# sandyresearch/chipmunk

Measured on AMD Instinct MI355X. Metric: DiT denoise steps/sec at fixed sparsity, higher is better.
Workload: dtype bf16

## Files before the change

chipmunk_amd/_native.py:

```python
from __future__ import annotations

import ctypes
import os

_HERE = os.path.dirname(os.path.abspath(__file__))
LIB_PATH = os.environ.get("CHIPMUNK_HIP_LIB") or os.path.join(_HERE, "lib", "libchipmunk_hip.so")

SYMBOLS = [
    "chipmunk_last_error", "chipmunk_abi_version", "chipmunk_set_option", "chipmunk_set_random_seed",
    "chipmunk_csp_attn", "chipmunk_csp_attn_out", "chipmunk_csp_128_attn", "chipmunk_dense_attn", "chipmunk_dense_colsum_attn",
    "chipmunk_csp_mlp_mm1", "chipmunk_csp_mlp_mm1_scatter", "chipmunk_csp_mlp_mm1_fp8", "chipmunk_csp_mlp_mm2_and_scatter_add", "chipmunk_csp_scatter_add", "chipmunk_csp_mlp_mm2",
    "chipmunk_csp_mlp_mm1_ragged", "chipmunk_csp_mlp_mm1_scatter_ragged", "chipmunk_csp_mlp_mm1_fp8_ragged", "chipmunk_csp_mlp_mm2_ragged",
    "chipmunk_csp_mlp_mm2_and_scatter_add_ragged", "chipmunk_csp_scatter_add_ragged", "chipmunk_block_mean_ragged", "chipmunk_transpose16_pitched",
    "chipmunk_csp_mlp_mm1_batched", "chipmunk_csp_mlp_mm1_scatter_batched", "chipmunk_csp_mlp_mm1_fp8_batched", "chipmunk_csp_mlp_mm2_batched",
    "chipmunk_csp_mlp_mm2_and_scatter_add_batched", "chipmunk_csp_scatter_add_batched",
    "chipmunk_csp_mlp_mm1_glu", "chipmunk_csp_mlp_mm1_glu_batched", "chipmunk_csp_mlp_mm1_glu_fp8", "chipmunk_csp_mlp_mm1_glu_fp8_batched",
    "chipmunk_csp_mlp_mm1_act", "chipmunk_csp_mlp_mm1_act_batched", "chipmunk_csp_mlp_mm1_fp8_act", "chipmunk_csp_mlp_mm1_fp8_act_batched",
    "chipmunk_csp_mlp_mm2_w8", "chipmunk_csp_mlp_mm2_w8_batched",
    "chipmunk_csp_mlp_mm1_w8", "chipmunk_csp_mlp_mm1_w8_batched", "chipmunk_csp_mlp_mm1_w8_gm", "chipmunk_w8_linear",
    "chipmunk_csp_mlp_mm1_fp8_act_rs", "chipmunk_csp_mlp_mm1_fp8_act_rs_batched", "chipmunk_quantize_fp8_rowwise",
    "chipmunk_csp_mlp_mm1_act_gm", "chipmunk_csp_mlp_mm1_fp8_act_gm", "chipmunk_csp_mlp_mm1_fp8_act_rs_gm", "chipmunk_csp_mlp_mm1_glu_gm",
    "chipmunk_csp_mlp_mm1_glu_fp8_gm", "chipmunk_csp_scatter_add_gm", "chipmunk_transpose16_groups",
    "chipmunk_topk_indices", "chipmunk_topk_delta_indices", "chipmunk_topk_indices_p", "chipmunk_topk_delta_indices_p", "chipmunk_topk_group_delta_indices", "chipmunk_topk_group_delta_indices_p", "chipmunk_topk_mask", "chipmunk_topk_mask_p", "chipmunk_dense_colsum_topk_mask_p_strided", "chipmunk_mask_to_indices", "chipmunk_mask_to_sorted_indices", "chipmunk_packed_mask_to_indices", "chipmunk_mask_row_counts", "chipmunk_mask_to_ragged_indices", "chipmunk_copy_indices",
    "chipmunk_bitpack", "chipmunk_bitunpack", "chipmunk_transpose16", "chipmunk_block_mean", "chipmunk_quantize_fp8", "chipmunk_gather_rows", "chipmunk_qkv_split_norm", "chipmunk_split_heads_rownorm", "chipmunk_dense_colsum_topk_mask", "chipmunk_dense_attn_strided", "chipmunk_csp_attn_out_ragged", "chipmunk_compact_indices", "chipmunk_residual_ln_modulate", "chipmunk_residual_ln_modulate_f32", "chipmunk_dense_colsum_attn_strided", "chipmunk_dense_colsum_topk_mask_strided", "chipmunk_release_scratch", "chipmunk_big_scratch_fallbacks",
    "chipmunk_dense_attn_varlen", "chipmunk_dense_colsum_attn_varlen", "chipmunk_dense_colsum_topk_mask_varlen",
    "chipmunk_dense_colsum_topk_mask_p_varlen", "chipmunk_topk_mask_varlen", "chipmunk_topk_mask_p_varlen",
    "chipmunk_host_alloc", "chipmunk_host_free", "chipmunk_copy_d2h_async", "chipmunk_copy_h2d_async", "chipmunk_host_bytes",
]

_lib = None


def lib() -> ctypes.CDLL:
    global _lib
    if _lib is None:
        if not os.path.exists(LIB_PATH):
            raise ImportError(
                f"{LIB_PATH} is missing: build it with `python -m chipmunk_amd.build` (hipcc --offload-arch=gfx950). "
                "chipmunk_amd has no CPU fallback.")
        _lib = ctypes.CDLL(LIB_PATH)
        _lib.chipmunk_last_error.restype = ctypes.c_char_p
        _lib.chipmunk_abi_version.restype = ctypes.c_int
        vp, i, d = ctypes.c_void_p, ctypes.c_int, ctypes.c_double
        if hasattr(_lib, "chipmunk_topk_group_delta_indices"):
            _lib.chipmunk_topk_group_delta_indices.argtypes = [vp, vp, i, vp, vp, i, i, i, i, d, i, d, vp]
            _lib.chipmunk_topk_group_delta_indices_p.argtypes = [vp, vp, i, vp, vp, i, i, i, i, d, d, d, i, d, vp]
        for item in filter(None, os.environ.get("CHIPMUNK_AMD_OPTIONS", "").split(",")):
            name, _, val = item.partition("=")
            if _lib.chipmunk_set_option(name.strip().encode(), int(val)) != 0:
                raise ValueError(f"CHIPMUNK_AMD_OPTIONS: {_lib.chipmunk_last_error().decode()}")
    return _lib


def last_error() -> str:
    return lib().chipmunk_last_error().decode()


def check(rc: int, what: str) -> None:
    if rc != 0:
# ... 59 lines not shown
```

chipmunk_amd/csrc/attn.hip:

```cpp
#include "common.h"
#include "attn_params.h"
#include <type_traits>

namespace {

constexpr int QG = 192;
constexpr int QW = 48;
constexpr int KVT = 32;
constexpr int NST = 4;
constexpr int KRING = 8;
constexpr int HD = 128;
constexpr int TILE_BYTES = KVT * HD * 2;
constexpr float SCALE_LOG2E = 0.08838834764f * 1.44269504089f;
constexpr int NSTV = NST + 1;
constexpr int KEY_RING_OFF = (NST + NSTV) * TILE_BYTES;
constexpr int CS_OFF = KEY_RING_OFF + KRING * 256;
constexpr int ATTN_LDS_BYTES = CS_OFF + 2 * 2 * 4 * KVT * 4;

__device__ __forceinline__ f32x4 mfma16(bf16x8 a, bf16x8 b, f32x4 c) {
    return __builtin_amdgcn_mfma_f32_16x16x32_bf16(a, b, c, 0, 0, 0);
}

#ifdef ATTN_PROF
__device__ unsigned long long g_attn_prof[8 * 8];
// ... 1217 lines not shown
    if (use_colsum64(B, H, Nq, Nk)) return chipmunk_colsum64_launch(p, st);
    return launch_attn<false, false, false, true>(p, st);
}

extern "C" int chipmunk_dense_colsum_attn_strided(const void *q, const void *k, const void *v, const int64_t q_strides[3],
                                                  const int64_t k_strides[3], const int64_t v_strides[3], const float *pin,
                                                  void *o, const int64_t *o_strides, void *cs, float *l, int B, int H, int Nq,
                                                  int Nk, int cs_stride, void *stream) {
    return dense_colsum_attn_impl(q, k, v, q_strides, k_strides, v_strides, pin, o, o_strides, cs, l, nullptr, B, H, Nq, Nk, cs_stride,
                                  stream);
}

extern "C" int chipmunk_dense_colsum_attn_varlen(const void *q, const void *k, const void *v, const int64_t q_strides[3],
                                                 const int64_t k_strides[3], const int64_t v_strides[3], const float *pin,
                                                 void *o, const int64_t *o_strides, void *cs, float *l, const int32_t *k_lens, int B,
                                                 int H, int Nq, int Nk, int cs_stride, void *stream) {
    return dense_colsum_attn_impl(q, k, v, q_strides, k_strides, v_strides, pin, o, o_strides, cs, l, k_lens, B, H, Nq, Nk, cs_stride,
                                  stream);
}

extern "C" int chipmunk_dense_colsum_attn(const void *q, const void *k, const void *v, const int64_t q_strides[3],
                                          const int64_t k_strides[3], const int64_t v_strides[3], const float *pin,
                                          void *o, void *cs, float *l, int B, int H, int Nq, int Nk, int cs_stride,
                                          void *stream) {
    return chipmunk_dense_colsum_attn_strided(q, k, v, q_strides, k_strides, v_strides, pin, o, nullptr, cs, l, B, H, Nq, Nk,
                                              cs_stride, stream);
}

static int dense_colsum_topk_mask_impl(const void *q, const void *k, const void *v, const int64_t q_strides[3],
                                       const int64_t k_strides[3], const int64_t v_strides[3], const float *pin, void *o,
                                       const int64_t *o_strides, float *l, int B, int H, int Nq, int Nk, const void *static_mask,
                                       int64_t static_stride, int static_rows, const void *group_flags, void *mask,
                                       int topk, double random_amount, bool mass, double top_p, int k_min, void *stream,
                                       const int32_t *klens = nullptr) {
    if (int e = check_common(q, k, v, o, B, H, Nq, Nk)) return e;
    CM_CHECK(l && pin && mask, "dense_colsum_topk_mask: p / l / mask missing");
    if (int e = check_strides(q_strides, "q")) return e;
    if (int e = check_strides(k_strides, "k")) return e;
    if (int e = check_strides(v_strides, "v")) return e;
    hipStream_t st = (hipStream_t)stream;
    if (!use_dense64(B, H, Nq, Nk) || chipmunk_get_option("attn_fused_colsum") == 2 || (Nk & 3) || Nk > CHIPMUNK_TOPK_MASK_MAX_N)
        return CHIPMUNK_ERR_UNSUPPORTED;
    AttnParams p = {};
    p.q = (const uint16_t *)q, p.k = (const uint16_t *)k, p.v = (const uint16_t *)v, p.o = (uint16_t *)o;
    for (int i = 0; i < 3; ++i) p.qs[i] = q_strides[i], p.ks[i] = k_strides[i], p.vs[i] = v_strides[i];
    CM_CHECK((int64_t)Nk * p.ks[2] * 2 < (1ll << 32) && (int64_t)Nk * p.vs[2] * 2 < (1ll << 32),
             "attention: one head's K or V spans more than 4 GiB (32-bit DMA offsets)");
    if (int e = output_strides(p.os, o_strides, H, Nq)) return e;
    p.l_out = l, p.p_in = pin, p.cs = nullptr, p.cs_stride = 0, p.klens = klens;
    p.B = B, p.H = H, p.Nq = Nq, p.Nk = Nk, p.G = (Nq + QG - 1) / QG;
    p.o_scale = 1.f;
    uint16_t *part = (uint16_t *)chipmunk_big_scratch(st, chipmunk_colsum_part_bytes(B, H, Nq, Nk));
    if (!part) return CHIPMUNK_ERR_UNSUPPORTED;
    if (int e = chipmunk_dense64_colsum_launch(p, part, st)) return e;
    const int nrb = ((Nq + 255) / 256) * 2;
    if (mass)
        return chipmunk_topk_mask_p_parts(part, chipmunk_colsum_part_stride(Nk), nrb, p.G, Nq, static_mask, static_stride, static_rows, group_flags, mask,
                                          B * H * p.G, Nk, topk, top_p, k_min, random_amount, st, klens, H * p.G);
    return chipmunk_topk_mask_parts(part, chipmunk_colsum_part_stride(Nk), nrb, p.G, Nq, static_mask, static_stride, static_rows, group_flags, mask, B * H * p.G, Nk,
                                    topk, random_amount, st, klens, H * p.G);
}

extern "C" int chipmunk_dense_colsum_topk_mask_strided(const void *q, const void *k, const void *v, const int64_t q_strides[3],
                                               const int64_t k_strides[3], const int64_t v_strides[3], const float *pin, void *o,
                                               const int64_t *o_strides, float *l, int B, int H, int Nq, int Nk, const void *static_mask,
                                               int64_t static_stride, int static_rows, const void *group_flags, void *mask,
                                               int topk, double random_amount, void *stream) {
    return dense_colsum_topk_mask_impl(q, k, v, q_strides, k_strides, v_strides, pin, o, o_strides, l, B, H, Nq, Nk, static_mask, static_stride,
                                       static_rows, group_flags, mask, topk, random_amount, false, 0.0, 0, stream);
}

extern "C" int chipmunk_dense_colsum_topk_mask_p_strided(const void *q, const void *k, const void *v, const int64_t q_strides[3],
                                                 const int64_t k_strides[3], const int64_t v_strides[3], const float *pin, void *o,
                                                 const int64_t *o_strides, float *l, int B, int H, int Nq, int Nk, const void *static_mask,
                                                 int64_t static_stride, int static_rows, const void *group_flags, void *mask,
                                                 int topk, double random_amount, double top_p, int k_min, void *stream) {
    CM_CHECK(top_p > 0.0 && top_p <= 1.0, "dense_colsum_topk_mask_p: top_p must be in (0, 1] (got %g)", top_p);
    CM_CHECK(k_min >= 0, "dense_colsum_topk_mask_p: k_min must be >= 0 (got %d)", k_min);
    return dense_colsum_topk_mask_impl(q, k, v, q_strides, k_strides, v_strides, pin, o, o_strides, l, B, H, Nq, Nk, static_mask, static_stride,
                                       static_rows, group_flags, mask, topk, random_amount, true, top_p, k_min, stream);
}

extern "C" int chipmunk_dense_colsum_topk_mask(const void *q, const void *k, const void *v, const int64_t q_strides[3],
                                               const int64_t k_strides[3], const int64_t v_strides[3], const float *pin, void *o,
                                               float *l, int B, int H, int Nq, int Nk, const void *static_mask,
                                               int64_t static_stride, int static_rows, const void *group_flags, void *mask,
                                               int topk, double random_amount, void *stream) {
    return chipmunk_dense_colsum_topk_mask_strided(q, k, v, q_strides, k_strides, v_strides, pin, o, nullptr, l, B, H, Nq, Nk,
                                                   static_mask, static_stride, static_rows, group_flags, mask, topk, random_amount,
                                                   stream);
}

extern "C" int chipmunk_dense_colsum_topk_mask_varlen(const void *q, const void *k, const void *v, const int64_t q_strides[3],
                                                      const int64_t k_strides[3], const int64_t v_strides[3], const float *pin, void *o,
                                                      const int64_t *o_strides, float *l, const int32_t *k_lens, int B, int H, int Nq,
                                                      int Nk, const void *static_mask, int64_t static_stride, int static_rows,
                                                      const void *group_flags, void *mask, int topk, double random_amount, void *stream) {
    return dense_colsum_topk_mask_impl(q, k, v, q_strides, k_strides, v_strides, pin, o, o_strides, l, B, H, Nq, Nk, static_mask, static_stride,
                                       static_rows, group_flags, mask, topk, random_amount, false, 0.0, 0, stream, k_lens);
}

extern "C" int chipmunk_dense_colsum_topk_mask_p_varlen(const void *q, const void *k, const void *v, const int64_t q_strides[3],
                                                        const int64_t k_strides[3], const int64_t v_strides[3], const float *pin, void *o,
                                                        const int64_t *o_strides, float *l, const int32_t *k_lens, int B, int H, int Nq,
                                                        int Nk, const void *static_mask, int64_t static_stride, int static_rows,
                                                        const void *group_flags, void *mask, int topk, double random_amount, double top_p,
                                                        int k_min, void *stream) {
    CM_CHECK(top_p > 0.0 && top_p <= 1.0, "dense_colsum_topk_mask_p: top_p must be in (0, 1] (got %g)", top_p);
    CM_CHECK(k_min >= 0, "dense_colsum_topk_mask_p: k_min must be >= 0 (got %d)", k_min);
    return dense_colsum_topk_mask_impl(q, k, v, q_strides, k_strides, v_strides, pin, o, o_strides, l, B, H, Nq, Nk, static_mask, static_stride,
                                       static_rows, group_flags, mask, topk, random_amount, true, top_p, k_min, stream, k_lens);
}
```

chipmunk_amd/csrc/attn_params.h:

```cpp
#pragma once
#include <stdint.h>
#include <hip/hip_runtime.h>

struct AttnParams {
    const uint16_t *q, *k, *v;
    uint16_t *o;
    const uint16_t *o_in;
    int64_t qs[3], ks[3], vs[3], os[3];
    const int32_t *indices, *counts;
    const int64_t *idx_off;
    float *l_out;
    const float *p_in;
    uint16_t *cs;
    int cs_stride;
    int B, H, Nq, Nk, G, idx_stride;
    float o_scale;
    int split_full, nsplit;
    float *ws;
    int32_t *tickets;
    const int32_t *plan;
    int xcd_chunks;
    const float *kmax;
    uint16_t *cs_part;
    int cs_pstride;
    int probe;
    const int32_t *klens;
};

__device__ __forceinline__ int item_nk(const int32_t *klens, int b, int Nk) {
    if (!klens) return Nk;
    const int n = klens[b];
    return n < 1 ? 1 : (n < Nk ? n : Nk);
}


int chipmunk_csp64_launch(const AttnParams &p, int inplace, int grid, hipStream_t stream);
int chipmunk_dense64_colsum_launch(const AttnParams &p, uint16_t *part, hipStream_t stream);
int chipmunk_topk_mask_parts(const uint16_t *part, int part_stride, int nrb, int groups_per_bh, int Nq, const void *static_mask, int64_t static_stride,
                             int static_rows, const void *group_flags, void *mask, int rows, int n, int k, double random_amount,
                             hipStream_t stream, const int32_t *klens = nullptr, int seq_rows = 0);
int chipmunk_topk_mask_p_parts(const uint16_t *part, int part_stride, int nrb, int groups_per_bh, int Nq, const void *static_mask, int64_t static_stride,
                               int static_rows, const void *group_flags, void *mask, int rows, int n, int k, double top_p, int k_min,
                               double random_amount, hipStream_t stream, const int32_t *klens = nullptr, int seq_rows = 0);
size_t chipmunk_colsum_part_bytes(int B, int H, int Nq, int Nk);
int chipmunk_colsum_part_stride(int Nk);
int chipmunk_colsum64_launch(const AttnParams &p, hipStream_t stream);
int chipmunk_csp96_launch(const AttnParams &p, int inplace, int grid, hipStream_t stream);
const float *chipmunk_knorm_max(const uint16_t *k, const int64_t ks[3], int B, int H, int Nk, hipStream_t stream, const int32_t *klens = nullptr);

__host__ __device__ inline int colsum_part_rows(int j, int nwg, int &r0, int &r1) {
    const int a = (3 * j) >> 2, w0 = 3 * j - 4 * a;
    r0 = 2 * a + (w0 ? 1 : 0);
    r1 = 2 * (a + 1);
    return (w0 >= 2 && a + 1 < nwg) ? 2 : 1;
}

struct IndexRow {
    const int32_t *ptr;
    int width;
};
__device__ __forceinline__ IndexRow index_row(const AttnParams &p, int64_t item) {
    if (p.idx_off) {
        const int64_t o = p.idx_off[item];
        return {p.indices + o, (int)(p.idx_off[item + 1] - o)};
    }
    return {p.indices + item * p.idx_stride, p.idx_stride};
}
```

chipmunk_amd/csrc/indexed_io.hip:

```cpp
#include "common.h"
#include "attn_params.h"

namespace {

__device__ __forceinline__ uint32_t wave_incl_scan(uint32_t x) {
    x += (uint32_t)__builtin_amdgcn_update_dpp(0, (int)x, 0x111, 0xf, 0xf, true);
    x += (uint32_t)__builtin_amdgcn_update_dpp(0, (int)x, 0x112, 0xf, 0xf, true);
    x += (uint32_t)__builtin_amdgcn_update_dpp(0, (int)x, 0x114, 0xf, 0xf, true);
    x += (uint32_t)__builtin_amdgcn_update_dpp(0, (int)x, 0x118, 0xf, 0xf, true);
    x += (uint32_t)__builtin_amdgcn_update_dpp(0, (int)x, 0x142, 0xa, 0xf, false);
    x += (uint32_t)__builtin_amdgcn_update_dpp(0, (int)x, 0x143, 0xc, 0xf, false);
    return x;
}
struct M2IParams {
    const uint8_t *mask;
    int32_t *indices;
    int32_t *counts;
    int n, pad_n, multiple_of;
    const int64_t *offsets;
};

template <bool PACKED, bool SORTED = false, bool RAGGED = false>
__global__ __launch_bounds__(256) void mask_to_indices_kernel(const M2IParams p) {
    extern __shared__ __attribute__((aligned(16))) unsigned char smem[];
// ... 190 lines not shown
};

template <bool PACKED>
__global__ __launch_bounds__(256) void mask_row_counts_kernel(const RowCountParams p) {
    const int lane = threadIdx.x & 63;
    const int64_t row = (int64_t)blockIdx.x * 4 + (threadIdx.x >> 6);
    if (row >= p.rows) return;
    const int nbytes = PACKED ? p.n >> 3 : p.n;
    const uint8_t *src = p.mask + (PACKED ? (row * p.n) >> 3 : row * p.n);
    auto set_in_byte = [](uint32_t b) { return PACKED ? (uint32_t)__popc(b) : (uint32_t)(b != 0); };
    auto set_in_word = [](uint32_t x) {
        if constexpr (!PACKED) x = (x | (x >> 1) | (x >> 2) | (x >> 3) | (x >> 4) | (x >> 5) | (x >> 6) | (x >> 7)) & 0x01010101u;
        return (uint32_t)__popc(x);
    };
    const int head = min(nbytes, (int)((16 - ((uintptr_t)src & 15)) & 15));
    uint32_t cnt = lane < head ? set_in_byte(src[lane]) : 0u;
    const int nvec = (nbytes - head) >> 4;
    const u32x4 *vec = (const u32x4 *)(src + head);
#pragma unroll 4
    for (int i = lane; i < nvec; i += 64) {
        const u32x4 x = vec[i];
        cnt += set_in_word(x[0]) + set_in_word(x[1]) + set_in_word(x[2]) + set_in_word(x[3]);
    }
    const int tail = head + (nvec << 4) + lane;
    if (tail < nbytes) cnt += set_in_byte(src[tail]);
    const int64_t kept = (uint32_t)__builtin_amdgcn_readlane((int)wave_incl_scan(cnt), 63);
    if (lane == 0) {
        const int64_t padded = ((kept + p.multiple_of - 1) / p.multiple_of) * p.multiple_of;
        p.counts[row] = (int32_t)padded;
        p.lengths[row] = (min(padded, (int64_t)p.pad_n) + 31) / 32 * 32;
    }
}

struct TopkParams {
    const void *act;
    void *cache;
    int32_t *indices;
    int32_t *counts;
    int rows, cols, multiple_of;
    float quantile, random_amount;
    uint32_t salt;
    int group_rows, src_rows, groups;
};

template <typename T>
__device__ __forceinline__ float load_as_float(const T *p, int i);
template <>
__device__ __forceinline__ float load_as_float<uint16_t>(const uint16_t *p, int i) { return bf16_bits_to_f32(p[i]); }
template <>
__device__ __forceinline__ float load_as_float<_Float16>(const _Float16 *p, int i) { return (float)p[i]; }
template <>
__device__ __forceinline__ float load_as_float<float>(const float *p, int i) { return p[i]; }

template <typename T>
__device__ __forceinline__ float round_to(float x);
template <>
__device__ __forceinline__ float round_to<uint16_t>(float x) { return round_bf16(x); }
template <>
__device__ __forceinline__ float round_to<_Float16>(float x) { return (float)(_Float16)x; }
template <>
__device__ __forceinline__ float round_to<float>(float x) { return x; }

__device__ __forceinline__ float hash_uniform(uint32_t row, uint32_t col, uint32_t salt) {
    uint32_t x = (row * 0x9E3779B9u ^ (col + 0x7F4A7C15u) * 0x85EBCA6Bu) + salt * 0xC2B2AE35u;
    x ^= x >> 16, x *= 0x7feb352du, x ^= x >> 15, x *= 0x846ca68bu, x ^= x >> 16;
    return (float)(x >> 8) * (1.0f / 16777216.0f);
// ... 359 lines not shown
    CM_CHECK(mask && indices && (RAGGED ? (const void *)offsets : (const void *)counts), "mask_to_indices: null pointer");
    CM_CHECK(rows >= 0 && n > 0 && pad_n >= n && multiple_of > 0, "mask_to_indices: bad sizes rows=%lld n=%d pad_n=%d multiple_of=%d",
             (long long)rows, n, pad_n, multiple_of);
    CM_CHECK(rows < (1ll << 31), "mask_to_indices: too many rows");
    if (PACKED) CM_CHECK(n % 8 == 0, "packed_mask_to_indices: n must be a multiple of 8 (got %d)", n);
    const size_t lds = m2i_lds_bytes(n, SORTED);
    CM_CHECK(lds <= 160 * 1024, "mask_to_indices: row length %d needs %zu B of LDS (> 160 KiB)", n, lds);
    if (rows == 0) return CHIPMUNK_OK;
    auto kern = mask_to_indices_kernel<PACKED, SORTED, RAGGED>;
    if (lds > 64 * 1024) (void)hipFuncSetAttribute((const void *)kern, hipFuncAttributeMaxDynamicSharedMemorySize, (int)lds);
    M2IParams p = {(const uint8_t *)mask, indices, counts, n, pad_n, multiple_of, offsets};
    hipLaunchKernelGGL(kern, dim3((unsigned)rows), dim3(256), lds, (hipStream_t)stream, p);
    CM_LAUNCH_CHECK();
    return CHIPMUNK_OK;
}


struct TopkMaskParams {
    const uint16_t *cs;
    const uint8_t *stat;
    const uint8_t *groups;
    uint8_t *mask;
    int64_t cs_stride, stat_stride;
    int rows, n, k, stat_rows;
    float random_amount;
    uint32_t salt;
    const uint16_t *parts;
    int64_t pstride;
    int nrb, ngroups, nq;
    float top_p;
    int k_min;
    const int32_t *klens;
    int seq_rows;
};

__device__ __forceinline__ int topk_mask_row_len(const TopkMaskParams &p, int row) {
    if (!p.klens) return p.n;
    const int v = p.klens[row / p.seq_rows];
    return v < 1 ? 1 : (v < p.n ? v : p.n);
}
struct RowCut {
    int tid, step;
    uint32_t keep0, keep1;
};
__device__ __forceinline__ RowCut row_cut(int nv) {
    const int rem = nv & 3;
    RowCut c;
    c.tid = rem ? ((nv - 1) >> 2) & 1023 : -1;
    c.step = (nv - 1) >> 12;
    c.keep0 = rem == 1 ? 0xffffu : 0xffffffffu;
    c.keep1 = rem == 3 ? 0xffffu : (rem ? 0u : 0xffffffffu);
    return c;
}

__device__ __forceinline__ float key_value(uint32_t key) { return __uint_as_float((key ^ 0x8000u) << 16); }
__device__ __forceinline__ void add_mass2(float &m, uint32_t kw, float flo) {
    const uint32_t kx = kw ^ 0x80008000u;
    const float a = __uint_as_float(kx << 16), b = __uint_as_float(kx & 0xffff0000u);
    m += a >= flo ? a : 0.f;
    m += b >= flo ? b : 0.f;
}

__device__ __forceinline__ int topp_count(float total, float target, float above, int gt, int eq, uint32_t thr, int k, int k_min) {
    int kp = 0;
    if (total > 0.f && target > 0.f) {
        const float v = key_value(thr);
        float t = __builtin_ceilf((target - above) / v);
        t = t >= 1.f ? t : 1.f;
        kp = gt + (t < (float)eq ? (int)t : eq);
    }
    const int s = kp > k_min ? kp : k_min;
    return s < k ? s : k;
}

__device__ __forceinline__ uint32_t bf16_key(uint32_t u) {
    return (u & 0x8000u) ? (~u & 0xffffu) : (u | 0x8000u);
}

template <int KPT, bool ALIGNED, bool PARTS = false, bool MASS = false>
__global__ __launch_bounds__(1024) void topk_mask_kernel(const TopkMaskParams p) {
    constexpr int NV = KPT / 4;
    __shared__ int wave_cnt[16];
    const int tid = threadIdx.x, lane = tid & 63, w = tid >> 6;
    const int row = blockIdx.x;
    const int n = p.n;
    const int nv = topk_mask_row_len(p, row);
    const uint16_t *x = nullptr;
    int prow = 1;
    int64_t row1 = 0;
    if constexpr (PARTS) {
        const int bh = row / p.ngroups, g = row - bh * p.ngroups;
        int r0, r1;
        prow = colsum_part_rows(g, p.nrb / 2, r0, r1);
        x = p.parts + ((int64_t)bh * p.nrb + r0) * p.pstride;
        row1 = (int64_t)(r1 - r0) * p.pstride;
    } else {
        x = p.cs + (int64_t)row * p.cs_stride;
    }
    const uint32_t lane_off8 = 8u * (uint32_t)tid;
    const uint32_t lane_off4 = 4u * (uint32_t)tid;
    uint32_t key[NV][2];
    constexpr int LB = NV % 10 == 0 ? 10 : (NV % 8 == 0 ? 8 : (NV % 6 == 0 ? 6 : 4));
    static_assert(NV % LB == 0, "NV must split into whole load batches");
#pragma unroll
    for (int j0 = 0; j0 < NV; j0 += LB) {
        uint32_t raw[LB][2];
#pragma unroll
        for (int jj = 0; jj < LB; ++jj) {
            const int c = 4 * tid + 4096 * (j0 + jj);
            uint32_t v0 = 0xffffffffu, v1 = 0xffffffffu;
            if constexpr (ALIGNED) {
                if (c < nv) {
                    const u32x2 v = *(const u32x2 *)((const unsigned char *)(x + 4096 * (j0 + jj)) + lane_off8);
// ... 142 lines not shown
                uint32_t kw = key[j][h];
                asm volatile("" : "+v"(kw));
                gt += ((kw & 0xffffu) > thr ? 1 : 0) + ((kw >> 16) > thr ? 1 : 0);
            }
        ties_to_take = k - block_count(gt);
    }
    int my_ties = 0;
    if (ties_to_take > 0) {
#pragma unroll
        for (int j = 0; j < NV; ++j)
#pragma unroll
            for (int h = 0; h < 2; ++h) {
                uint32_t kw = key[j][h];
                asm volatile("" : "+v"(kw));
                my_ties += ((kw & 0xffffu) == thr ? 1 : 0) + ((kw >> 16) == thr ? 1 : 0);
            }
    }
    int tie_budget = 0;
    {
        int incl = my_ties;
#pragma unroll
        for (int d = 1; d < 64; d <<= 1) {
            const int o = __shfl_up(incl, d);
            if (lane >= d) incl += o;
        }
        if (lane == 63) wave_cnt[w] = incl;
        __syncthreads();
        int before = incl - my_ties;
#pragma unroll
        for (int i = 0; i < 16; ++i) before += i < w ? wave_cnt[i] : 0;
        __syncthreads();
        tie_budget = ties_to_take - before;
    }
    uint8_t *out = p.mask + (int64_t)row * n;
    const uint8_t *st = p.stat ? p.stat + (int64_t)(row % p.stat_rows) * p.stat_stride : nullptr;
    const bool rnd = active && p.random_amount > 0.f;
    auto combined4 = [&](int c0, uint32_t &v0, uint32_t &v1) {
        const u32x2 v = *(const u32x2 *)(x + c0);
        v0 = v[0], v1 = v[1];
        if constexpr (PARTS) {
            float a0 = __uint_as_float(v0 << 16), a1 = __uint_as_float(v0 & 0xffff0000u);
            float a2 = __uint_as_float(v1 << 16), a3 = __uint_as_float(v1 & 0xffff0000u);
            if (prow == 2) {
                const u32x2 y = *(const u32x2 *)(x + row1 + c0);
                a0 += __uint_as_float(y[0] << 16), a1 += __uint_as_float(y[0] & 0xffff0000u);
                a2 += __uint_as_float(y[1] << 16), a3 += __uint_as_float(y[1] & 0xffff0000u);
            }
            v0 = pack_bf16x2(a0, a1), v1 = pack_bf16x2(a2, a3);
        }
    };
    uint32_t first = x[0];
    if constexpr (PARTS) {
        uint32_t f0, f1;
        combined4(0, f0, f1);
        first = f0 & 0xffffu;
    }
    const uint32_t salt = p.salt ^ (first * 0x27D4EB2Fu);
    const int nsteps = (n + 4095) / 4096;
    auto emit = [&](auto keyed, int c, uint32_t v0, uint32_t v1, uint32_t sb) {
        uint32_t bytes = 0;
        if constexpr (decltype(keyed)::value) asm volatile("" : "+v"(v0), "+v"(v1));
#pragma unroll
        for (int e = 0; e < 4; ++e) {
            const uint32_t half = ((e < 2 ? v0 : v1) >> (16 * (e & 1))) & 0xffffu;
            const uint32_t kv = decltype(keyed)::value ? half : bf16_key(half);
            bool keep = kv > thr;
            const bool tie = kv == thr && tie_budget > 0 && c + e < nv;
            tie_budget -= tie ? 1 : 0;
            keep = keep || tie;
            if (rnd && !keep) keep = hash_uniform(row, c + e, salt) < p.random_amount;
            keep = keep || ((sb >> (8 * e)) & 0xffu) != 0;
            keep = keep && c + e < nv;
            bytes |= (keep ? 1u : 0u) << (8 * e);
        }
        if constexpr (ALIGNED) {
            *(uint32_t *)(out + c) = bytes;
        } else {
#pragma unroll
            for (int e = 0; e < 4; ++e)
                if (c + e < n) out[c + e] = (uint8_t)(bytes >> (8 * e));
        }
    };
    if constexpr (ALIGNED) {
        constexpr int OB = 5;
#pragma unroll
        for (int j0 = 0; j0 < NV; j0 += OB) {
            uint32_t sbv[OB];
#pragma unroll
            for (int jj = 0; jj < OB; ++jj) {
                const int c = 4 * tid + 4096 * (j0 + jj);
                sbv[jj] = (j0 + jj < NV && st && c < n) ? *(const uint32_t *)(st + c) : 0u;
            }
            __builtin_amdgcn_sched_barrier(0);
#pragma unroll
            for (int jj = 0; jj < OB; ++jj) {
                if constexpr (true) {
                    const int c = 4 * tid + 4096 * (j0 + jj);
                    if (j0 + jj < NV && c < n) emit(std::integral_constant<int, 1>{}, c, key[(j0 + jj) < NV ? (j0 + jj) : 0][0], key[(j0 + jj) < NV ? (j0 + jj) : 0][1], sbv[jj]);
                    asm volatile("" ::: "memory");
                }
            }
            __builtin_amdgcn_sched_barrier(0);
        }
    } else {
        for (int j = 0; j < nsteps; ++j) {
            const int c = 4 * tid + 4096 * j;
            if (c >= n) break;
            uint32_t v0 = 0, v1 = 0, sb = 0;
#pragma unroll
            for (int e = 0; e < 4; ++e) {
                const uint32_t u = c + e < nv ? x[c + e] : 0xffffu;
                if (e < 2) v0 |= u << (16 * e);
                else v1 |= u << (16 * (e - 2));
                if (st && c + e < n) sb |= (uint32_t)st[c + e] << (8 * e);
            }
            emit(std::integral_constant<int, 0>{}, c, v0, v1, sb);
        }
    }
}

__device__ __forceinline__ uint32_t bf16_key2(uint32_t u) {
    uint32_t s;
    const uint32_t fifteen2 = 0x000f000fu;
    asm("v_pk_ashrrev_i16 %0, %1, %2" : "=v"(s) : "v"(fifteen2), "v"(u));
    return u ^ (s | 0x80008000u);
}

template <bool ALIGNED, bool PARTS, bool MASS = false>
__global__ __launch_bounds__(1024) void topk_mask_stream_kernel(const TopkMaskParams p) {
    __shared__ int wave_cnt[16];
    const int tid = threadIdx.x, lane = tid & 63, w = tid >> 6;
    const int row = blockIdx.x;
    const int n = p.n;
    const int nv = topk_mask_row_len(p, row);
    const uint16_t *x = nullptr;
    int prow = 1;
    int64_t row1 = 0;
    if constexpr (PARTS) {
        const int bh = row / p.ngroups, g = row - bh * p.ngroups;
        int r0, r1;
        prow = colsum_part_rows(g, p.nrb / 2, r0, r1);
        x = p.parts + ((int64_t)bh * p.nrb + r0) * p.pstride;
        row1 = (int64_t)(r1 - r0) * p.pstride;
    } else {
        x = p.cs + (int64_t)row * p.cs_stride;
    }
    const uint32_t lane_off8 = 8u * (uint32_t)tid;
    const int nsteps = (n + 4095) / 4096;
    const bool active = p.groups == nullptr || p.groups[row] != 0;
    int k = p.k < nv ? p.k : nv;
    const RowCut rc = row_cut(nv);
    const int cut_step = ALIGNED && tid == rc.tid ? rc.step : -1;
    bool select = active && k > 0;
    const bool rnd = active && p.random_amount > 0.f;

    auto combined4 = [&](int c0, uint32_t &v0, uint32_t &v1) {
        const u32x2 v = *(const u32x2 *)(x + c0);
        v0 = v[0], v1 = v[1];
        if constexpr (PARTS) {
            if (prow == 2) {
                float a0 = __uint_as_float(v0 << 16), a1 = __uint_as_float(v0 & 0xffff0000u);
                float a2 = __uint_as_float(v1 << 16), a3 = __uint_as_float(v1 & 0xffff0000u);
// ... 152 lines not shown
        for (int j0 = 0; j0 < nsteps; j0 += U) {
            uint32_t kw[U][2];
#pragma unroll
            for (int jj = 0; jj < U; ++jj) load_raw(j0 + jj, kw[jj][0], kw[jj][1]);
#pragma unroll
            for (int jj = 0; jj < U; ++jj) {
                to_keys(kw[jj][0], kw[jj][1]);
#pragma unroll
                for (int h = 0; h < 2; ++h) {
                    const uint32_t lo = kw[jj][h] & 0xffffu, hi = kw[jj][h] >> 16;
                    gt += (lo > thr ? 1 : 0) + (hi > thr ? 1 : 0);
                    my_ties += (lo == thr ? 1 : 0) + (hi == thr ? 1 : 0);
                }
            }
        }
        ties_to_take = k - block_count(gt);
    }
    int tie_budget = 0;
    {
        int incl = my_ties;
#pragma unroll
        for (int d = 1; d < 64; d <<= 1) {
            const int o = __shfl_up(incl, d);
            if (lane >= d) incl += o;
        }
        if (lane == 63) wave_cnt[w] = incl;
        __syncthreads();
        int before = incl - my_ties;
#pragma unroll
        for (int i = 0; i < 16; ++i) before += i < w ? wave_cnt[i] : 0;
        __syncthreads();
        tie_budget = ties_to_take - before;
    }
    uint8_t *out = p.mask + (int64_t)row * n;
    const uint8_t *st = p.stat ? p.stat + (int64_t)(row % p.stat_rows) * p.stat_stride : nullptr;
    for (int j0 = 0; j0 < nsteps; j0 += U) {
        uint32_t kw[U][2], sbv[U];
#pragma unroll
        for (int jj = 0; jj < U; ++jj) {
            const int c = 4 * tid + 4096 * (j0 + jj);
            kw[jj][0] = kw[jj][1] = 0;
            if (select) load_raw(j0 + jj, kw[jj][0], kw[jj][1]);
            sbv[jj] = 0;
            if constexpr (ALIGNED) {
                if (st && c < n) sbv[jj] = *(const uint32_t *)(st + c);
            } else if (st) {
#pragma unroll
                for (int e = 0; e < 4; ++e)
                    if (c + e < n) sbv[jj] |= (uint32_t)st[c + e] << (8 * e);
            }
        }
#pragma unroll
        for (int jj = 0; jj < U; ++jj) {
            const int c = 4 * tid + 4096 * (j0 + jj);
            if (c >= n) continue;
            if (select) to_keys(kw[jj][0], kw[jj][1]);
            uint32_t bytes = 0;
#pragma unroll
            for (int e = 0; e < 4; ++e) {
                const uint32_t kv = (kw[jj][e >> 1] >> (16 * (e & 1))) & 0xffffu;
                bool keep = kv > thr;
                const bool tie = kv == thr && tie_budget > 0 && c + e < nv;
                tie_budget -= tie ? 1 : 0;
                keep = keep || tie;
                if (rnd && !keep) keep = hash_uniform(row, c + e, salt) < p.random_amount;
                keep = keep || ((sbv[jj] >> (8 * e)) & 0xffu) != 0;
                keep = keep && c + e < nv;
                bytes |= (keep ? 1u : 0u) << (8 * e);
            }
            if constexpr (ALIGNED) {
                *(uint32_t *)(out + c) = bytes;
            } else {
#pragma unroll
                for (int e = 0; e < 4; ++e)
                    if (c + e < n) out[c + e] = (uint8_t)(bytes >> (8 * e));
            }
        }
    }
}

}

extern "C" int chipmunk_mask_to_indices(const void *mask, int32_t *indices, int32_t *counts, int64_t rows, int n,
                                        int pad_n, int multiple_of, void *stream) {
    return launch_m2i<false>(mask, indices, counts, rows, n, pad_n, multiple_of, stream);
}

extern "C" int chipmunk_packed_mask_to_indices(const void *packed, int32_t *indices, int32_t *counts, int64_t rows,
                                               int n, int pad_n, int multiple_of, void *stream) {
    return launch_m2i<true>(packed, indices, counts, rows, n, pad_n, multiple_of, stream);
}

struct TopkGroups {
    int batches, src_rows, group_rows;
    int groups() const { return (src_rows + group_rows - 1) / group_rows; }
};
static int check_topk_groups(const char *who, const TopkGroups &gs, const void *activation, const void *cache, const int32_t *indices,
                             const int32_t *counts, int cols, int *rows) {
    CM_CHECK(activation && cache && indices && counts, "%s: null pointer", who);
    CM_CHECK(cols >= 1024, "%s: cols >= 1024 required (the quantile is taken over the first 1024 columns); got cols=%d", who, cols);
    CM_CHECK(gs.group_rows >= 1 && gs.group_rows <= 64, "%s: rows_per_group must be in [1, 64] (got %d)", who, gs.group_rows);
    CM_CHECK(gs.batches >= 0 && gs.src_rows >= 1, "%s: B >= 0 and rows >= 1 required; got B=%d rows=%d", who, gs.batches, gs.src_rows);
    CM_CHECK((int64_t)gs.batches * gs.groups() < (1ll << 31), "%s: too many groups (B=%d times %d)", who, gs.batches, gs.groups());
    *rows = gs.batches * gs.groups();
    return CHIPMUNK_OK;
}

static int launch_topk(const void *activation, void *cache, int dtype, int32_t *indices, int32_t *counts, int rows,
                       int cols, double sparsity_amount, int multiple_of, double random_amount, void *stream,
                       const TopkGroups *gs = nullptr) {
// ... 56 lines not shown
        case CHIPMUNK_DTYPE_FP16: LAUNCH_TOPK_P(_Float16); break;
        case CHIPMUNK_DTYPE_FP32: LAUNCH_TOPK_P(float); break;
        default: CM_CHECK(false, "%s: unsupported dtype code %d", who, dtype);
    }
#undef LAUNCH_TOPK_P
    CM_LAUNCH_CHECK();
    return CHIPMUNK_OK;
}

extern "C" int chipmunk_mask_to_sorted_indices(const void *mask, int packed, int32_t *indices, int32_t *counts,
                                               int64_t rows, int n, int pad_n, int multiple_of, void *stream) {
    return packed ? launch_m2i<true, true>(mask, indices, counts, rows, n, pad_n, multiple_of, stream)
                  : launch_m2i<false, true>(mask, indices, counts, rows, n, pad_n, multiple_of, stream);
}

extern "C" int chipmunk_mask_row_counts(const void *mask, int packed, int32_t *counts, int64_t *lengths, int64_t rows, int n,
                                        int pad_n, int multiple_of, void *stream) {
    CM_CHECK(mask && counts && lengths, "mask_row_counts: null pointer");
    CM_CHECK(rows >= 0 && n > 0 && pad_n >= n && multiple_of > 0, "mask_row_counts: bad sizes rows=%lld n=%d pad_n=%d multiple_of=%d",
             (long long)rows, n, pad_n, multiple_of);
    CM_CHECK(rows < (1ll << 31), "mask_row_counts: too many rows");
    CM_CHECK(!packed || n % 8 == 0, "mask_row_counts: n must be a multiple of 8 for a packed mask (got %d)", n);
    const size_t lds = m2i_lds_bytes(n, true);
    CM_CHECK(lds <= 160 * 1024, "mask_to_indices: row length %d needs %zu B of LDS (> 160 KiB)", n, lds);
    if (rows == 0) return CHIPMUNK_OK;
    RowCountParams p = {(const uint8_t *)mask, counts, lengths, rows, n, pad_n, multiple_of};
    const dim3 grid((unsigned)((rows + 3) / 4));
    if (packed) hipLaunchKernelGGL(mask_row_counts_kernel<true>, grid, dim3(256), 0, (hipStream_t)stream, p);
    else hipLaunchKernelGGL(mask_row_counts_kernel<false>, grid, dim3(256), 0, (hipStream_t)stream, p);
    CM_LAUNCH_CHECK();
    return CHIPMUNK_OK;
}

extern "C" int chipmunk_mask_to_ragged_indices(const void *mask, int packed, int sorted, const int64_t *offsets, int32_t *flat,
                                               int64_t rows, int n, int multiple_of, void *stream) {
    if (packed) return sorted ? launch_m2i<true, true, true>(mask, flat, nullptr, rows, n, n, multiple_of, stream, offsets)
                              : launch_m2i<true, false, true>(mask, flat, nullptr, rows, n, n, multiple_of, stream, offsets);
    return sorted ? launch_m2i<false, true, true>(mask, flat, nullptr, rows, n, n, multiple_of, stream, offsets)
                  : launch_m2i<false, false, true>(mask, flat, nullptr, rows, n, n, multiple_of, stream, offsets);
}

extern "C" int chipmunk_topk_indices(const void *activation, int dtype, int32_t *indices, int32_t *counts, int rows,
                                     int cols, double sparsity_amount, int multiple_of, double random_amount,
                                     void *stream) {
    return launch_topk(activation, nullptr, dtype, indices, counts, rows, cols, sparsity_amount, multiple_of,
                       random_amount, stream);
}

extern "C" int chipmunk_topk_delta_indices(const void *activation, void *cache, int dtype, int32_t *indices,
                                           int32_t *counts, int rows, int cols, double sparsity_amount,
                                           int multiple_of, double random_amount, void *stream) {
    CM_CHECK(cache != nullptr, "topk_delta_indices: cache missing");
    return launch_topk(activation, cache, dtype, indices, counts, rows, cols, sparsity_amount, multiple_of,
                       random_amount, stream);
}

extern "C" int chipmunk_topk_indices_p(const void *activation, int dtype, int32_t *indices, int32_t *counts, int rows, int cols,
                                       double sparsity_amount, double top_p, double min_keys, int multiple_of,
                                       double random_amount, void *stream) {
    return launch_topk_p("topk_indices_p", activation, nullptr, dtype, indices, counts, rows, cols, sparsity_amount, top_p, min_keys,
                         multiple_of, random_amount, stream);
}

extern "C" int chipmunk_topk_delta_indices_p(const void *activation, void *cache, int dtype, int32_t *indices, int32_t *counts,
                                             int rows, int cols, double sparsity_amount, double top_p, double min_keys,
                                             int multiple_of, double random_amount, void *stream) {
// ... 79 lines not shown
template <typename V>
__global__ __launch_bounds__(256) void gather_rows_kernel(const V *src, V *dst, const int32_t *map, int64_t n_out,
                                                          int64_t n_src, int64_t cpr, int64_t total) {
    for (int64_t idx = (int64_t)blockIdx.x * 256 + threadIdx.x; idx < total; idx += (int64_t)gridDim.x * 256) {
        const int64_t row = idx / cpr, c = idx - row * cpr;
        const int64_t o = row / n_out, r = row - o * n_out;
        dst[idx] = src[(o * n_src + map[r]) * cpr + c];
    }
}

extern "C" int chipmunk_gather_rows(const void *src, void *dst, const int32_t *map, int64_t outer, int64_t n_src,
                                    int64_t n_out, int64_t row_bytes, void *stream) {
    CM_CHECK(src && dst && map, "gather_rows: null pointer");
    CM_CHECK(outer >= 0 && n_src > 0 && n_out >= 0 && row_bytes > 0, "gather_rows: bad sizes");
    if (outer == 0 || n_out == 0) return CHIPMUNK_OK;
    hipStream_t s = (hipStream_t)stream;
    const uintptr_t align = (uintptr_t)src | (uintptr_t)dst | (uintptr_t)row_bytes;
#define LAUNCH_GATHER(V)                                                                                              \
    do {                                                                                                              \
        const int64_t cpr = row_bytes / (int64_t)sizeof(V), total = outer * n_out * cpr;                               \
        const int64_t blocks = (total + 255) / 256;                                                                    \
        hipLaunchKernelGGL((gather_rows_kernel<V>), dim3((unsigned)(blocks > 65536 * 16 ? 65536 * 16 : blocks)),       \
                           dim3(256), 0, s, (const V *)src, (V *)dst, map, n_out, n_src, cpr, total);                  \
    } while (0)
    if ((align & 15) == 0) LAUNCH_GATHER(u32x4);
    else if ((align & 3) == 0) LAUNCH_GATHER(uint32_t);
    else if ((align & 1) == 0) LAUNCH_GATHER(uint16_t);
    else LAUNCH_GATHER(uint8_t);
#undef LAUNCH_GATHER
    CM_LAUNCH_CHECK();
    return CHIPMUNK_OK;
}

template <bool MASS>
static int topk_mask_parts_impl(const uint16_t *part, int part_stride, int nrb, int groups_per_bh, int Nq, const void *static_mask, int64_t static_stride,
                                int static_rows, const void *group_flags, void *mask, int rows, int n, int k, double random_amount,
                                double top_p, int k_min, hipStream_t s, const int32_t *klens, int seq_rows) {
    CM_CHECK(!klens || seq_rows > 0, "topk_mask_parts: k_lens without the rows per sequence");
    CM_CHECK(part && mask && rows >= 0 && n > 0 && (n & 3) == 0 && n <= CHIPMUNK_TOPK_MASK_MAX_N && k >= 0 && part_stride >= n && (part_stride & 3) == 0, "topk_mask_parts: bad arguments");
    CM_CHECK(!static_mask || (static_rows > 0 && static_stride >= n && (static_stride & 3) == 0 && ((uintptr_t)static_mask & 3) == 0),
             "topk_mask_parts: bad static mask geometry");
    CM_CHECK(((uintptr_t)mask & 3) == 0 && ((uintptr_t)part & 7) == 0, "topk_mask_parts: unaligned buffers");
    if (rows == 0) return CHIPMUNK_OK;
    TopkMaskParams p = {nullptr, (const uint8_t *)static_mask, (const uint8_t *)group_flags, (uint8_t *)mask, 0, static_stride,
                        rows, n, k, static_mask ? static_rows : 1, (float)random_amount,
                        random_amount > 0.0 ? chipmunk_next_random_salt() : 0u};
    p.parts = part, p.pstride = part_stride, p.nrb = nrb, p.ngroups = groups_per_bh, p.nq = Nq;
    p.top_p = (float)top_p, p.k_min = k_min;
    p.klens = klens, p.seq_rows = seq_rows;
    if (n > 1024 * 120 || chipmunk_get_option("topk_mask_stream") == 1) hipLaunchKernelGGL((topk_mask_stream_kernel<true, true, MASS>), dim3(rows), dim3(1024), 0, s, p);
    else if (n <= 1024 * 16) hipLaunchKernelGGL((topk_mask_kernel<16, true, true, MASS>), dim3(rows), dim3(1024), 0, s, p);
    else if (n <= 1024 * 48) hipLaunchKernelGGL((topk_mask_kernel<48, true, true, MASS>), dim3(rows), dim3(1024), 0, s, p);
    else hipLaunchKernelGGL((topk_mask_kernel<120, true, true, MASS>), dim3(rows), dim3(1024), 0, s, p);
    CM_LAUNCH_CHECK();
    return CHIPMUNK_OK;
}

int chipmunk_topk_mask_parts(const uint16_t *part, int part_stride, int nrb, int groups_per_bh, int Nq, const void *static_mask, int64_t static_stride,
                             int static_rows, const void *group_flags, void *mask, int rows, int n, int k, double random_amount,
                             hipStream_t s, const int32_t *klens, int seq_rows) {
    return topk_mask_parts_impl<false>(part, part_stride, nrb, groups_per_bh, Nq, static_mask, static_stride, static_rows, group_flags, mask, rows, n, k,
                                       random_amount, 0.0, 0, s, klens, seq_rows);
}

int chipmunk_topk_mask_p_parts(const uint16_t *part, int part_stride, int nrb, int groups_per_bh, int Nq, const void *static_mask, int64_t static_stride,
                               int static_rows, const void *group_flags, void *mask, int rows, int n, int k, double top_p, int k_min,
                               double random_amount, hipStream_t s, const int32_t *klens, int seq_rows) {
    CM_CHECK(top_p > 0.0 && top_p <= 1.0 && k_min >= 0, "topk_mask_p_parts: top_p must be in (0, 1] and k_min >= 0 (got %g, %d)", top_p, k_min);
    return topk_mask_parts_impl<true>(part, part_stride, nrb, groups_per_bh, Nq, static_mask, static_stride, static_rows, group_flags, mask, rows, n, k,
                                      random_amount, top_p, k_min, s, klens, seq_rows);
}

__global__ __launch_bounds__(256) void qkv_split_norm_kernel(const uint16_t *qkv, int64_t row_stride, const uint16_t *qw,
                                                             const uint16_t *kw, uint16_t *q, uint16_t *k, uint16_t *v, int64_t n,
                                                             int H, float eps, int64_t segments, const float *fcos, const float *fsin,
                                                             int64_t rope_rows) {
    const int l15 = threadIdx.x & 15;
    u32x4 wq = {0x3f803f80u, 0x3f803f80u, 0x3f803f80u, 0x3f803f80u}, wk = wq;
    if (qw) wq = *(const u32x4 *)(qw + l15 * 8);
    if (kw) wk = *(const u32x4 *)(kw + l15 * 8);
    for (int64_t seg = ((int64_t)blockIdx.x * 256 + threadIdx.x) >> 4; seg < segments; seg += ((int64_t)gridDim.x * 256) >> 4) {
        const int64_t tok = seg / (3 * H);
        const int rem = (int)(seg - tok * 3 * H), which = rem / H, h = rem - which * H;
        u32x4 x = *(const u32x4 *)(qkv + tok * row_stride + (int64_t)rem * 128 + l15 * 8);
        uint16_t *dst = (which == 0 ? q : which == 1 ? k : v) + ((int64_t)h * n + tok) * 128 + l15 * 8;
        if (which < 2) {
            float f[8], ss = 0.f;
#pragma unroll
            for (int e = 0; e < 4; ++e) {
                f[2 * e] = __uint_as_float(x[e] << 16), f[2 * e + 1] = __uint_as_float(x[e] & 0xffff0000u);
                ss = __builtin_fmaf(f[2 * e], f[2 * e], ss);
                ss = __builtin_fmaf(f[2 * e + 1], f[2 * e + 1], ss);
            }
            ss = row16_sum(ss);
            const float r = 1.0f / __builtin_sqrtf(ss * (1.0f / 128.0f) + eps);
            const u32x4 w = which == 0 ? wq : wk;
#pragma unroll
            for (int e = 0; e < 4; ++e) {
                float a = f[2 * e] * r, b = f[2 * e + 1] * r;
                round_bf16_pair(a, b);
                x[e] = pack_bf16x2(a * __uint_as_float(w[e] << 16), b * __uint_as_float(w[e] & 0xffff0000u));
            }
            if (fcos && tok < rope_rows) {
// ... 36 lines not shown
                          double random_amount, double top_p, int k_min, void *stream, const int32_t *klens = nullptr, int seq_rows = 0) {
    CM_CHECK(cs && mask, "topk_mask: null pointer");
    CM_CHECK(!klens || (seq_rows > 0 && rows % seq_rows == 0), "topk_mask: %d rows are no whole sequences of %d rows", rows, seq_rows);
    CM_CHECK(rows >= 0 && n > 0 && k >= 0, "topk_mask: bad sizes (rows=%d n=%d k=%d)", rows, n, k);
    CM_CHECK(cs_stride >= n, "topk_mask: cs row stride %lld < n %d", (long long)cs_stride, n);
    CM_CHECK(n <= CHIPMUNK_TOPK_MASK_MAX_N, "topk_mask: rows of more than %d columns are not supported (got %d)", CHIPMUNK_TOPK_MASK_MAX_N, n);
    CM_CHECK(!static_mask || (static_rows > 0 && static_stride >= n), "topk_mask: bad static mask geometry");
    CM_CHECK(random_amount >= 0.0 && random_amount <= 1.0, "topk_mask: random_amount must be in [0,1]");
    if (rows == 0) return CHIPMUNK_OK;
    TopkMaskParams p = {(const uint16_t *)cs, (const uint8_t *)static_mask, (const uint8_t *)group_flags, (uint8_t *)mask,
                        cs_stride, static_stride, rows, n, k, static_mask ? static_rows : 1, (float)random_amount,
                        random_amount > 0.0 ? chipmunk_next_random_salt() : 0u};
    p.top_p = (float)top_p, p.k_min = k_min;
    p.klens = klens, p.seq_rows = seq_rows;
    hipStream_t s = (hipStream_t)stream;
    const bool aligned = n % 4 == 0 && (((uintptr_t)cs) & 7) == 0 && (cs_stride * 2) % 8 == 0 && (((uintptr_t)mask) & 3) == 0 &&
                         (!static_mask || ((((uintptr_t)static_mask) & 3) == 0 && static_stride % 4 == 0));
#define LAUNCH_TM(KPT)                                                                                       \
    do {                                                                                                     \
        if (aligned) hipLaunchKernelGGL((topk_mask_kernel<KPT, true, false, MASS>), dim3(rows), dim3(1024), 0, s, p);     \
        else hipLaunchKernelGGL((topk_mask_kernel<KPT, false, false, MASS>), dim3(rows), dim3(1024), 0, s, p);            \
    } while (0)
    if (n > 1024 * 120 || chipmunk_get_option("topk_mask_stream") == 1) {
        if (aligned) hipLaunchKernelGGL((topk_mask_stream_kernel<true, false, MASS>), dim3(rows), dim3(1024), 0, s, p);
        else hipLaunchKernelGGL((topk_mask_stream_kernel<false, false, MASS>), dim3(rows), dim3(1024), 0, s, p);
    } else if (n <= 1024 * 16) LAUNCH_TM(16);
    else if (n <= 1024 * 48) LAUNCH_TM(48);
    else LAUNCH_TM(120);
#undef LAUNCH_TM
    CM_LAUNCH_CHECK();
    return CHIPMUNK_OK;
}

extern "C" int chipmunk_topk_mask(const void *cs, int64_t cs_stride, const void *static_mask, int64_t static_stride,
                                  int static_rows, const void *group_flags, void *mask, int rows, int n, int k,
                                  double random_amount, void *stream) {
    return topk_mask_impl<false>(cs, cs_stride, static_mask, static_stride, static_rows, group_flags, mask, rows, n, k, random_amount, 0.0, 0, stream);
}

extern "C" int chipmunk_topk_mask_p(const void *cs, int64_t cs_stride, const void *static_mask, int64_t static_stride,
                                    int static_rows, const void *group_flags, void *mask, int rows, int n, int k,
                                    double random_amount, double top_p, int k_min, void *stream) {
    CM_CHECK(top_p > 0.0 && top_p <= 1.0, "topk_mask_p: top_p must be in (0, 1] (got %g)", top_p);
    CM_CHECK(k_min >= 0, "topk_mask_p: k_min must be >= 0 (got %d)", k_min);
    return topk_mask_impl<true>(cs, cs_stride, static_mask, static_stride, static_rows, group_flags, mask, rows, n, k, random_amount, top_p, k_min, stream);
}

extern "C" int chipmunk_topk_mask_varlen(const void *cs, int64_t cs_stride, const void *static_mask, int64_t static_stride,
                                         int static_rows, const void *group_flags, void *mask, const int32_t *k_lens, int seq_rows, int rows,
                                         int n, int k, double random_amount, void *stream) {
    return topk_mask_impl<false>(cs, cs_stride, static_mask, static_stride, static_rows, group_flags, mask, rows, n, k, random_amount, 0.0, 0, stream,
                                 k_lens, seq_rows);
}

extern "C" int chipmunk_topk_mask_p_varlen(const void *cs, int64_t cs_stride, const void *static_mask, int64_t static_stride,
                                           int static_rows, const void *group_flags, void *mask, const int32_t *k_lens, int seq_rows, int rows,
                                           int n, int k, double random_amount, double top_p, int k_min, void *stream) {
    CM_CHECK(top_p > 0.0 && top_p <= 1.0, "topk_mask_p: top_p must be in (0, 1] (got %g)", top_p);
    CM_CHECK(k_min >= 0, "topk_mask_p: k_min must be >= 0 (got %d)", k_min);
    return topk_mask_impl<true>(cs, cs_stride, static_mask, static_stride, static_rows, group_flags, mask, rows, n, k, random_amount, top_p, k_min,
                                stream, k_lens, seq_rows);
}

extern "C" int chipmunk_compact_indices(const int32_t *indices, int64_t idx_stride, const int32_t *counts, const int64_t *offsets,
                                        int32_t *flat, int64_t rows, void *stream) {
    CM_CHECK(indices && counts && offsets && flat, "compact_indices: null pointer");
// ... 9 lines not shown
```

chipmunk_amd/csrc/torch_registry.cpp:

```cpp
#include <ATen/ATen.h>
#include <ATen/hip/impl/HIPStreamMasqueradingAsCUDA.h>
#include <Python.h>
#include <c10/core/DeviceGuard.h>
#include <torch/library.h>

#include <vector>

#include "../../include/chipmunk_hip.h"

extern "C" {
PyObject *PyInit_cuda(void) {
    static struct PyModuleDef module_def = {PyModuleDef_HEAD_INIT, "cuda", NULL, -1, NULL};
    return PyModule_Create(&module_def);
}
}

namespace chipmunk {
namespace {

void *cur_stream(const at::Tensor &t) {
    return (void *)c10::hip::getCurrentHIPStreamMasqueradingAsCUDA(t.device().index()).stream();
}
void check(int rc, const char *op) { TORCH_CHECK(rc == 0, "chipmunk::", op, ": ", chipmunk_last_error()); }

// ... 1081 lines not shown
    TORCH_CHECK(x.dim() >= 1 && x.size(-1) > 0 && x.size(-1) % 16 == 0 && x.size(-1) <= CHIPMUNK_QUANTIZE_ROWWISE_MAX_K,
                "quantize_fp8_rowwise: the last dimension must be a positive multiple of 16, at most ", CHIPMUNK_QUANTIZE_ROWWISE_MAX_K);
    x = x.contiguous();
    c10::DeviceGuard guard(x.device());
    const int64_t K = x.size(-1), rows = x.numel() / K;
    at::Tensor out = at::empty(x.sizes(), x.options().dtype(at::kFloat8_e4m3fn));
    at::Tensor recip = at::empty(x.sizes().slice(0, x.dim() - 1), x.options().dtype(at::kFloat));
    check(chipmunk_quantize_fp8_rowwise(x.data_ptr(), out.data_ptr(), recip.data_ptr<float>(), rows, (int)K, (float)max_value, cur_stream(x)),
          "quantize_fp8_rowwise");
    return {out, recip};
}

std::vector<at::Tensor> mask_to_sorted_indices(at::Tensor mask, at::IntArrayRef shape, int64_t multiple_of,
                                               int64_t pad_to_multiple_of) {
    CHECK_DEV(mask);
    const bool packed = mask.scalar_type() == at::kByte;
    TORCH_CHECK(packed || mask.scalar_type() == at::kBool, "mask must be bool, or uint8 bit-packed with a shape");
    mask = mask.contiguous();
    std::vector<int64_t> shp = packed ? shape.vec() : mask.sizes().vec();
    TORCH_CHECK(shp.size() == 4, "shape must be [b, h, m, n]");
    const int64_t b = shp[0], h = shp[1], m = shp[2], n = shp[3];
    if (packed) TORCH_CHECK(n % 8 == 0 && mask.numel() * 8 >= b * h * m * n, "bad packed mask");
    const int64_t pad_n = ((n + pad_to_multiple_of - 1) / pad_to_multiple_of) * pad_to_multiple_of;
    c10::DeviceGuard guard(mask.device());
    at::Tensor indices = at::empty({b, h, m, pad_n}, mask.options().dtype(at::kInt));
    at::Tensor counts = at::empty({b, h, m}, mask.options().dtype(at::kInt));
    check(chipmunk_mask_to_sorted_indices(mask.data_ptr(), packed ? 1 : 0, indices.data_ptr<int>(),
                                          counts.data_ptr<int>(), b * h * m, (int)n, (int)pad_n, (int)multiple_of,
                                          cur_stream(mask)),
          "mask_to_sorted_indices");
    return {indices, counts};
}

std::vector<at::Tensor> mask_to_ragged_indices(at::Tensor mask, at::IntArrayRef shape, int64_t multiple_of, int64_t pad_to_multiple_of,
                                               bool sorted) {
    CHECK_DEV(mask);
    const bool packed = mask.scalar_type() == at::kByte;
    TORCH_CHECK(packed || mask.scalar_type() == at::kBool, "mask must be bool, or uint8 bit-packed with a shape");
    TORCH_CHECK(multiple_of > 0 && pad_to_multiple_of > 0, "multiple_of and pad_to_multiple_of must be positive");
    mask = mask.contiguous();
    std::vector<int64_t> shp = packed ? shape.vec() : mask.sizes().vec();
    TORCH_CHECK(shp.size() == 4, "shape must be [b, h, m, n]");
    const int64_t b = shp[0], h = shp[1], m = shp[2], n = shp[3], rows = b * h * m;
    if (packed) TORCH_CHECK(n % 8 == 0 && mask.numel() * 8 >= rows * n, "bad packed mask");
    const int64_t pad_n = ((n + pad_to_multiple_of - 1) / pad_to_multiple_of) * pad_to_multiple_of;
    TORCH_CHECK(n > 0 && pad_n <= INT_MAX, "rows must have between 1 and 2^31 - 1 columns");
    c10::DeviceGuard guard(mask.device());
    at::Tensor counts = at::empty({b, h, m}, mask.options().dtype(at::kInt));
    at::Tensor len = at::empty({rows}, mask.options().dtype(at::kLong));
    check(chipmunk_mask_row_counts(mask.data_ptr(), packed ? 1 : 0, counts.data_ptr<int>(), len.data_ptr<int64_t>(), rows, (int)n,
                                   (int)pad_n, (int)multiple_of, cur_stream(mask)),
          "mask_to_ragged_indices");
    at::Tensor offsets = at::zeros({rows + 1}, len.options());
    if (rows) offsets.narrow(0, 1, rows).copy_(len.cumsum(0));
    const int64_t total = rows ? offsets[rows].item<int64_t>() : 0;
    at::Tensor flat = at::empty({total + 64}, counts.options());
    flat.narrow(0, total, 64).zero_();
    check(chipmunk_mask_to_ragged_indices(mask.data_ptr(), packed ? 1 : 0, sorted ? 1 : 0, offsets.data_ptr<int64_t>(), flat.data_ptr<int>(),
                                          rows, (int)n, (int)multiple_of, cur_stream(mask)),
          "mask_to_ragged_indices");
    return {flat, offsets, counts};
}

std::vector<at::Tensor> dense_colsum_attn_layout(at::Tensor q, at::Tensor k, at::Tensor v, at::Tensor p, bool token_major_o);
static at::Tensor topk_mask_impl(at::Tensor cs, int64_t k, bool mass, double top_p, int64_t k_min, double random_amount,
                                 const c10::optional<at::Tensor> &groups, const c10::optional<at::Tensor> &static_mask,
                                 const OptTensor &k_lens = c10::nullopt);
static std::vector<at::Tensor> dense_colsum_topk_mask_impl(at::Tensor q, at::Tensor k, at::Tensor v, at::Tensor p, int64_t k_top, bool mass, double top_p,
                                                           int64_t k_min, double random_amount, const c10::optional<at::Tensor> &groups,
                                                           const c10::optional<at::Tensor> &static_mask, bool token_major_o,
                                                           const OptTensor &k_lens = c10::nullopt) {
    const int32_t *kl = klens_ptr(k_lens, q, q.dim() == 4 ? q.size(0) : 0);
    if (mass) TORCH_CHECK(top_p > 0.0 && top_p <= 1.0 && k_min >= 0, "top_p must be in (0, 1] and k_min >= 0 (got ", top_p, ", ", k_min, ")");
    CHECK_DEV(q); CHECK_DEV(k); CHECK_DEV(v); CHECK_DEV(p);
    CHECK_BF16(q); CHECK_BF16(k); CHECK_BF16(v);
    const bool shapes_ok = q.dim() == 4 && k.dim() == 4 && v.dim() == 4 && q.size(3) == 128 && q.stride(3) == 1 && k.stride(3) == 1 &&
                           v.stride(3) == 1 && p.scalar_type() == at::kFloat && p.is_contiguous();
    if (shapes_ok) {
        const int64_t B = q.size(0), H = q.size(1), Nq = q.size(2), Nk = k.size(2), G = (Nq + 191) / 192;
        const void *st = nullptr, *gf = nullptr;
        int64_t st_stride = 0, st_rows = 1;
        at::Tensor stc, gfc;
        bool ok = p.numel() == B * H * Nq;
        if (ok && static_mask.has_value() && static_mask->defined()) {
            stc = *static_mask;
            ok = stc.is_cuda() && stc.scalar_type() == at::kBool && stc.dim() == 4 && stc.size(3) == Nk && stc.size(2) == G && stc.size(1) == H &&
                 (stc.size(0) == 1 || stc.size(0) == B) && stc.stride(3) == 1 && stc.stride(1) == G * stc.stride(2) &&
                 (stc.size(0) == 1 || stc.stride(0) == H * stc.stride(1));
            if (ok) st = stc.data_ptr(), st_stride = stc.stride(2), st_rows = stc.size(0) * H * G;
        }
        if (ok && groups.has_value() && groups->defined()) {
            gfc = *groups;
            ok = gfc.is_cuda() && gfc.scalar_type() == at::kBool && gfc.dim() == 4 && gfc.size(3) == 1 && gfc.size(2) == G && gfc.size(1) == H &&
                 (gfc.size(0) == 1 || gfc.size(0) == B);
// ... 83 lines not shown
        gf = gfc.data_ptr();
    }
    if (mass)
        check(chipmunk_topk_mask_p_varlen(cs.data_ptr(), cs.stride(2), st, st_stride, (int)st_rows, gf, mask.data_ptr(), kl, (int)(H * G),
                                          (int)rows, (int)N, (int)k, random_amount, top_p, (int)(k_min > N ? N : k_min), cur_stream(cs)),
              "topk_mask_p");
    else
        check(chipmunk_topk_mask_varlen(cs.data_ptr(), cs.stride(2), st, st_stride, (int)st_rows, gf, mask.data_ptr(), kl, (int)(H * G),
                                        (int)rows, (int)N, (int)k, random_amount, cur_stream(cs)),
              "topk_mask");
    return mask;
}

at::Tensor topk_mask_varlen(at::Tensor cs, at::Tensor k_lens, int64_t k, double random_amount, const c10::optional<at::Tensor> &groups,
                            const c10::optional<at::Tensor> &static_mask) {
    return topk_mask_impl(cs, k, false, 0.0, 0, random_amount, groups, static_mask, k_lens);
}

at::Tensor topk_mask_p_varlen(at::Tensor cs, at::Tensor k_lens, int64_t k, double top_p, int64_t k_min, double random_amount,
                              const c10::optional<at::Tensor> &groups, const c10::optional<at::Tensor> &static_mask) {
    return topk_mask_impl(cs, k, true, top_p, k_min, random_amount, groups, static_mask, k_lens);
}

at::Tensor topk_mask(at::Tensor cs, int64_t k, double random_amount, const c10::optional<at::Tensor> &groups,
                     const c10::optional<at::Tensor> &static_mask) {
    return topk_mask_impl(cs, k, false, 0.0, 0, random_amount, groups, static_mask);
}

at::Tensor topk_mask_p(at::Tensor cs, int64_t k, double top_p, int64_t k_min, double random_amount, const c10::optional<at::Tensor> &groups,
                       const c10::optional<at::Tensor> &static_mask) {
    return topk_mask_impl(cs, k, true, top_p, k_min, random_amount, groups, static_mask);
}

at::Tensor bitpack(at::Tensor mask) {
    TORCH_CHECK(mask.scalar_type() == at::kBool, "mask must be bool type");
    CHECK_DEV(mask);
    mask = mask.contiguous();
    c10::DeviceGuard guard(mask.device());
    at::Tensor packed = at::empty({(mask.numel() + 7) / 8}, mask.options().dtype(at::kByte));
    check(chipmunk_bitpack(mask.data_ptr(), packed.data_ptr(), mask.numel(), cur_stream(mask)), "bitpack");
    return packed;
}
at::Tensor bitunpack(at::Tensor packed, at::IntArrayRef shape) {
    TORCH_CHECK(packed.scalar_type() == at::kByte && packed.is_contiguous(), "packed must be a contiguous uint8 tensor");
    CHECK_DEV(packed);
    int64_t n = 1;
    for (auto d : shape) n *= d;
    TORCH_CHECK(packed.numel() * 8 >= n, "packed is too short for the given shape");
    c10::DeviceGuard guard(packed.device());
    at::Tensor mask = at::empty(shape, packed.options().dtype(at::kBool));
    check(chipmunk_bitunpack(packed.data_ptr(), mask.data_ptr(), n, cur_stream(packed)), "bitunpack");
    return mask;
}

std::vector<at::Tensor> qkv_split_norm(at::Tensor qkv, const c10::optional<at::Tensor> &q_weight, const c10::optional<at::Tensor> &k_weight,
                                       int64_t heads, double eps, const c10::optional<at::Tensor> &freqs_cos,
                                       const c10::optional<at::Tensor> &freqs_sin) {
    CHECK_DEV(qkv); CHECK_BF16(qkv);
    TORCH_CHECK(qkv.dim() == 2 && qkv.stride(1) == 1 && qkv.size(1) >= 3 * heads * 128, "qkv_split_norm: qkv must be [n, >= 3*heads*128] with a contiguous last dim");
    const void *qw = nullptr, *kw = nullptr;
    at::Tensor qwc, kwc;
    if (q_weight.has_value() && q_weight->defined()) { qwc = q_weight->contiguous(); CHECK_DEV(qwc); CHECK_BF16(qwc); TORCH_CHECK(qwc.numel() == 128); qw = qwc.data_ptr(); }
    if (k_weight.has_value() && k_weight->defined()) { kwc = k_weight->contiguous(); CHECK_DEV(kwc); CHECK_BF16(kwc); TORCH_CHECK(kwc.numel() == 128); kw = kwc.data_ptr(); }
    const int64_t n = qkv.size(0);
    const float *fc = nullptr, *fs = nullptr;
    int64_t rope_rows = 0;
// ... 102 lines not shown
    m.def("csp_attn_out(Tensor q, Tensor k, Tensor v, Tensor o_in, Tensor indices, Tensor indices_counts, int o_scale) -> Tensor");
    m.def("csp_mlp_mm1_scatter(Tensor a, Tensor b_colmajor, Tensor(c!) c, Tensor bias, Tensor(pa_cache_colmajor!) pa_cache_colmajor, Tensor indices, Tensor indices_counts) -> ()");
    m.def("csp_mlp_mm2(Tensor mma_a, Tensor mma_b, Tensor indices, Tensor counts, Tensor(mma_c!) mma_c) -> ()");
    m.def("csp_mlp_mm2_w8(Tensor mma_a, Tensor mma_b, Tensor scale_b, Tensor indices, Tensor counts, Tensor(mma_c!) mma_c) -> ()");
    m.def("csp_mlp_mm1_fp8(Tensor a, Tensor b, Tensor(c!) c, Tensor bias, Tensor(pa_cache_colmajor!) pa_cache_colmajor, Tensor indices, Tensor indices_counts, Tensor scale_a, Tensor scale_b, bool update_cache) -> ()");
    m.def("csp_mlp_mm1_fp8_scatter(Tensor a, Tensor b, Tensor(c!) c, Tensor bias, Tensor(pa_cache_colmajor!) pa_cache_colmajor, Tensor indices, Tensor indices_counts, Tensor scale_a, Tensor scale_b) -> ()");
    m.def("csp_mlp_mm1_glu(Tensor a, Tensor b_gate, Tensor b_up, Tensor(c!) c, Tensor? bias_gate, Tensor? bias_up, Tensor(pa_cache_colmajor!) pa_cache_colmajor, Tensor indices, Tensor indices_counts, str act, bool update_cache) -> ()");
    m.def("csp_mlp_mm1_glu_fp8(Tensor a, Tensor b_gate, Tensor b_up, Tensor(c!) c, Tensor? bias_gate, Tensor? bias_up, Tensor(pa_cache_colmajor!) pa_cache_colmajor, Tensor indices, Tensor indices_counts, Tensor scale_a, Tensor scale_b_gate, Tensor scale_b_up, str act, bool update_cache) -> ()");
    m.def("csp_mlp_mm1_act(Tensor a, Tensor b, Tensor(c!) c, Tensor? bias, Tensor(pa!) pa_cache, Tensor indices, Tensor counts, str act, bool update_cache) -> ()");
    m.def("csp_mlp_mm1_w8(Tensor a, Tensor b, Tensor scale_b, Tensor(c!) c, Tensor? bias, Tensor(pa!) pa_cache, Tensor indices, Tensor counts, str act, bool update_cache) -> ()");
    m.def("w8_linear(Tensor x, Tensor w, Tensor scale_b, Tensor? bias, Tensor(a!) y) -> ()");
    m.def("csp_mlp_mm1_fp8_act(Tensor a, Tensor b, Tensor(c!) c, Tensor? bias, Tensor(pa!) pa_cache, Tensor indices, Tensor counts, Tensor scale_a, Tensor scale_b, str act, int update_cache) -> ()");
    m.def("topk_delta_indices(Tensor activation, Tensor(cache!) cache, Tensor(indices!) indices, Tensor(counts!) counts, float sparsity_amount, int multiple_of, float random_amount) -> ()");
    m.def("topk_indices_p(Tensor activation, Tensor(indices!) indices, Tensor(counts!) counts, float sparsity_amount, float top_p, float min_keys, int multiple_of, float random_amount) -> ()");
    m.def("topk_delta_indices_p(Tensor activation, Tensor(cache!) cache, Tensor(indices!) indices, Tensor(counts!) counts, float sparsity_amount, float top_p, float min_keys, int multiple_of, float random_amount) -> ()");
    m.def("topk_group_delta_indices(Tensor activation, Tensor(cache!) cache, Tensor(indices!) indices, Tensor(counts!) counts, int rows_per_group, float sparsity_amount, int multiple_of, float random_amount) -> ()");
    m.def("topk_group_delta_indices_p(Tensor activation, Tensor(cache!) cache, Tensor(indices!) indices, Tensor(counts!) counts, int rows_per_group, float sparsity_amount, float top_p, float min_keys, int multiple_of, float random_amount) -> ()");
    m.def("packed_mask_to_indices(Tensor packed, int[] shape, int multiple_of, int pad_to_multiple_of) -> Tensor[]");
    m.def("mask_to_sorted_indices(Tensor mask, int[] shape, int multiple_of, int pad_to_multiple_of) -> Tensor[]");
    m.def("topk_mask(Tensor cs, int k, float random_amount, Tensor? groups, Tensor? static_mask) -> Tensor");
    m.def("dense_colsum_topk_mask(Tensor q, Tensor k, Tensor v, Tensor p, int k_top, float random_amount, Tensor? groups, Tensor? static_mask, bool token_major_o=False) -> Tensor[]");
    m.def("topk_mask_p(Tensor cs, int k, float top_p, int k_min, float random_amount, Tensor? groups, Tensor? static_mask) -> Tensor");
    m.def("dense_colsum_topk_mask_p(Tensor q, Tensor k, Tensor v, Tensor p, int k_top, float top_p, int k_min, float random_amount, Tensor? groups, Tensor? static_mask, bool token_major_o=False) -> Tensor[]");
    m.def("dense_attn_layout(Tensor q, Tensor k, Tensor v, bool token_major_o) -> Tensor[]");
    m.def("dense_colsum_attn_layout(Tensor q, Tensor k, Tensor v, Tensor p, bool token_major_o) -> Tensor[]");
    m.def("dense_attn_varlen(Tensor q, Tensor k, Tensor v, Tensor k_lens, bool token_major_o=False) -> Tensor[]");
    m.def("dense_colsum_attn_varlen(Tensor q, Tensor k, Tensor v, Tensor p, Tensor k_lens, bool token_major_o=False) -> Tensor[]");
    m.def("topk_mask_varlen(Tensor cs, Tensor k_lens, int k, float random_amount, Tensor? groups, Tensor? static_mask) -> Tensor");
    m.def("topk_mask_p_varlen(Tensor cs, Tensor k_lens, int k, float top_p, int k_min, float random_amount, Tensor? groups, Tensor? static_mask) -> Tensor");
    m.def("dense_colsum_topk_mask_varlen(Tensor q, Tensor k, Tensor v, Tensor p, Tensor k_lens, int k_top, float random_amount, Tensor? groups, Tensor? static_mask, bool token_major_o=False) -> Tensor[]");
    m.def("dense_colsum_topk_mask_p_varlen(Tensor q, Tensor k, Tensor v, Tensor p, Tensor k_lens, int k_top, float top_p, int k_min, float random_amount, Tensor? groups, Tensor? static_mask, bool token_major_o=False) -> Tensor[]");
    m.def("compact_indices(Tensor indices, Tensor counts) -> Tensor[]");
    m.def("mask_to_ragged_indices(Tensor mask, int[] shape, int multiple_of, int pad_to_multiple_of, bool sorted) -> Tensor[]");
    m.def("csp_attn_out_ragged(Tensor q, Tensor k, Tensor v, Tensor o_in, Tensor indices, Tensor offsets, Tensor indices_counts, int o_scale) -> Tensor");
    m.def("residual_ln_modulate(Tensor x, Tensor? y, Tensor? gate, Tensor shift, Tensor scale, float eps) -> Tensor[]");
    m.def("residual_ln_modulate_f32(Tensor x, Tensor? y, Tensor? gate, Tensor? shift, Tensor? scale, Tensor? weight, Tensor? bias, float eps) -> Tensor[]");
    m.def("transpose_last2(Tensor x) -> Tensor");
    m.def("transpose_last2_pitched(Tensor x, int ld) -> Tensor");
    m.def("transpose_to_groups(Tensor x) -> Tensor");
    m.def("csp_scatter_add_gm(Tensor packed, Tensor(unpacked_groups!) unpacked_groups, Tensor sp_inds, Tensor sp_counts) -> ()");
    m.def("block_mean(Tensor x, int mbm) -> Tensor");
    m.def("quantize_fp8(Tensor x, Tensor scale, float max_value) -> Tensor");
    m.def("quantize_fp8_rowwise(Tensor x, float max_value) -> Tensor[]");
    m.def("csp_mlp_mm1_fp8_act_rs(Tensor a, Tensor b, Tensor(c!) c, Tensor? bias, Tensor(pa!) pa_cache, Tensor indices, Tensor counts, Tensor scale_a, Tensor scale_b, str act, int update_cache) -> ()");
    m.def("bitpack(Tensor mask) -> Tensor");
    m.def("bitunpack(Tensor packed, int[] shape) -> Tensor");
    m.def("gather_rows(Tensor src, Tensor map) -> Tensor");
    m.def("qkv_split_norm(Tensor qkv, Tensor? q_weight, Tensor? k_weight, int heads, float eps, Tensor? freqs_cos=None, Tensor? freqs_sin=None) -> Tensor[]");
    m.def("split_heads_rownorm(Tensor x, int heads, int parts, Tensor? w0, Tensor? w1, Tensor? w2, int norm_mask, int rope_mask, float eps, Tensor? freqs_cos=None, Tensor? freqs_sin=None) -> Tensor[]");
}

TORCH_LIBRARY_IMPL(chipmunk, CUDA, m) {
    m.impl("qkv_split_norm", &qkv_split_norm);
    m.impl("split_heads_rownorm", &split_heads_rownorm);
    m.impl("csp_mlp_mm1_fp8_scatter", &csp_mlp_mm1_fp8_scatter);
    m.impl("dense_colsum_topk_mask", &dense_colsum_topk_mask);
    m.impl("dense_colsum_topk_mask_p", &dense_colsum_topk_mask_p);
    m.impl("csp_mlp_mm1", &csp_mlp_mm1);
    m.impl("csp_mlp_mm2_and_scatter_add", &csp_mlp_mm2_and_scatter_add);
    m.impl("copy_indices", &copy_indices);
    m.impl("topk_indices", &topk_indices);
    m.impl("csp_scatter_add", &csp_scatter_add);
    m.impl("mask_to_indices", &mask_to_indices);
    m.impl("csp_attn", &csp_attn);
    m.impl("csp_128_attn", &csp_128_attn);
    m.impl("dense_attn", &dense_attn);
    m.impl("dense_colsum_attn", &dense_colsum_attn);
    m.impl("compact_indices", &compact_indices);
    m.impl("residual_ln_modulate", &residual_ln_modulate);
    m.impl("residual_ln_modulate_f32", &residual_ln_modulate_f32);
    m.impl("csp_attn_out_ragged", &csp_attn_out_ragged);
    m.impl("dense_attn_varlen", &dense_attn_varlen);
    m.impl("dense_colsum_attn_varlen", &dense_colsum_attn_varlen);
    m.impl("topk_mask_varlen", &topk_mask_varlen);
    m.impl("topk_mask_p_varlen", &topk_mask_p_varlen);
    m.impl("dense_colsum_topk_mask_varlen", &dense_colsum_topk_mask_varlen);
    m.impl("dense_colsum_topk_mask_p_varlen", &dense_colsum_topk_mask_p_varlen);
    m.impl("dense_attn_layout", &dense_attn_layout);
    m.impl("dense_colsum_attn_layout", &dense_colsum_attn_layout);
    m.impl("csp_attn_out", &csp_attn_out);
    m.impl("csp_mlp_mm1_scatter", &csp_mlp_mm1_scatter);
    m.impl("csp_mlp_mm2", &csp_mlp_mm2);
    m.impl("csp_mlp_mm2_w8", &csp_mlp_mm2_w8);
    m.impl("csp_mlp_mm1_fp8", &csp_mlp_mm1_fp8);
    m.impl("csp_mlp_mm1_glu", &csp_mlp_mm1_glu);
    m.impl("csp_mlp_mm1_glu_fp8", &csp_mlp_mm1_glu_fp8);
    m.impl("csp_mlp_mm1_act", &csp_mlp_mm1_act);
    m.impl("csp_mlp_mm1_w8", &csp_mlp_mm1_w8);
    m.impl("w8_linear", &w8_linear);
    m.impl("csp_mlp_mm1_fp8_act", &csp_mlp_mm1_fp8_act);
    m.impl("topk_delta_indices", &topk_delta_indices);
    m.impl("topk_indices_p", &topk_indices_p);
    m.impl("topk_delta_indices_p", &topk_delta_indices_p);
    m.impl("topk_group_delta_indices", &topk_group_delta_indices);
    m.impl("topk_group_delta_indices_p", &topk_group_delta_indices_p);
    m.impl("packed_mask_to_indices", &packed_mask_to_indices);
    m.impl("mask_to_sorted_indices", &mask_to_sorted_indices);
    m.impl("mask_to_ragged_indices", &mask_to_ragged_indices);
    m.impl("topk_mask", &topk_mask);
    m.impl("topk_mask_p", &topk_mask_p);
    m.impl("transpose_last2", &transpose_last2);
    m.impl("transpose_last2_pitched", &transpose_last2_pitched);
    m.impl("transpose_to_groups", &transpose_to_groups);
    m.impl("csp_scatter_add_gm", &csp_scatter_add_gm);
    m.impl("block_mean", &block_mean);
    m.impl("quantize_fp8", &quantize_fp8);
    m.impl("quantize_fp8_rowwise", &quantize_fp8_rowwise);
    m.impl("csp_mlp_mm1_fp8_act_rs", &csp_mlp_mm1_fp8_act_rs);
    m.impl("bitpack", &bitpack);
    m.impl("bitunpack", &bitunpack);
    m.impl("gather_rows", &gather_rows);
}

}
```

chipmunk_amd/modules/attn.py:

```python
from __future__ import annotations

from typing import Optional, Tuple

import torch
import torch.nn.functional as F
from torch import Tensor, nn

from .. import ops
from ..ops.voxel import get_local_indices_with_text
from ..util.config import GLOBAL_CONFIG, amd_key
from ..util.layer_counter import LayerCounter
from ..util.storage import AttnStorage
from ..util.storage.offloaded_tensor import release_kept_offloaded, release_resident, reserve_kept_offloaded, reserve_resident

singleton_static_mask: Optional[Tensor] = None
singleton_video_query_groups: Optional[Tensor] = None


def _cdiv(a: int, b: int) -> int:
    return (a + b - 1) // b


def _dense_attn_raw(q: Tensor, k: Tensor, v: Tensor, token_major_o: bool, k_lens: Optional[Tensor] = None):
    if k_lens is not None:
        return torch.ops.chipmunk.dense_attn_varlen(q, k, v, k_lens, token_major_o)
    return torch.ops.chipmunk.dense_attn_layout(q, k, v, True) if token_major_o else torch.ops.chipmunk.dense_attn(q, k, v)


def _valid_keys(k_lens: Tensor, n: int) -> Tensor:
    return (torch.arange(n, device=k_lens.device)[None, :] < k_lens[:, None])[:, None, None, :]


def _cap_counts(counts: Tensor, k_lens: Optional[Tensor]) -> Tensor:
    return counts if k_lens is None else torch.minimum(counts, k_lens.view(-1, 1, 1).to(counts.dtype))


class SparseDiffAttn(nn.Module):
    def __init__(self, layer_num: int, layer_counter: LayerCounter, storage_slot: int = 0, query_group_offset: int = 0):
        super().__init__()
        self.layer_num = layer_num
        self.layer_counter = layer_counter
        self.query_group_offset = query_group_offset
        self.storage = AttnStorage(layer_num, init_names=["indices", "out_cache"], slot=storage_slot)
        self.mask_shape = [None] * GLOBAL_CONFIG["num_model_invocations_per_inference_step"]
        self._unpacked = [None] * GLOBAL_CONFIG["num_model_invocations_per_inference_step"]

    def initialize_static_mask(self, seq_shape: Tuple, txt_len: int, local_heads_num: int, device: torch.device):
        if len(seq_shape) == 2:
            raise NotImplementedError("Not yet implemented for 2D sequences")
        tt, th, tw = seq_shape
        cfg = GLOBAL_CONFIG["attn"]
        n_video = tt * th * tw
        topk = int(cfg["top_keys"] * n_video)
        lv = cfg["local_voxels"]
        mask, _, _ = get_local_indices_with_text(vid_shape=(tt, th, tw), txt_len=txt_len, voxel_shape=(4, 6, 8),
                                                 local_shape=(lv, lv, lv), rk=cfg["random_keys"], device=device)
        if cfg["local_1d_window"] > 0:
            window = int(cfg["local_1d_window"] * n_video)
            for qg in range(n_video // 192):
                centre = qg * 192 + 96
                mask[qg, max(0, centre - window // 2):min(n_video, centre + window // 2)] = True
        mask = mask[None, None, :, :].expand(1, local_heads_num, -1, -1).contiguous()
        sparse_groups = (mask.sum(dim=-1, keepdim=True) + topk) < (n_video + txt_len)
        global singleton_static_mask, singleton_video_query_groups
        singleton_static_mask = mask
        singleton_video_query_groups = sparse_groups

    def _static(self, heads: int, qg: int, n: int):
        g0 = self.query_group_offset
        assert heads <= singleton_static_mask.shape[1] or singleton_static_mask.shape[1] == 1, (
            f"this module serves {heads} heads but initialize_static_mask() built {singleton_static_mask.shape[1]} head planes "
            "(local_heads_num): build the static mask for the largest head chunk")
        h = min(heads, singleton_static_mask.shape[1])
        return (singleton_static_mask[:, :h, g0:g0 + qg, :n], singleton_video_query_groups[:, :h, g0:g0 + qg, :])

    @staticmethod
    def _top_p(n_keys: int, multiple_of: int):
        top_p = float(amd_key("attn", "top_p"))
        if top_p == 0.0:
            return 0.0, 0
        if not 0.0 < top_p <= 1.0:
            raise ValueError(f"attn.top_p must be in [0, 1] (got {top_p})")
        if not GLOBAL_CONFIG["attn"]["should_compress_indices"]:
            raise ValueError("attn.top_p needs attn.should_compress_indices: without it the layer stores fixed-width torch.topk indices, "
                             "which cannot hold a key count per query group")
        return top_p, int(multiple_of * round((float(amd_key("attn", "top_p_min_keys")) * n_keys) / multiple_of))

    def random_and_topk(self, cs: Tensor, topk: int, top_p: float = 0.0, k_min: int = 0, k_lens: Optional[Tensor] = None) -> Tensor:
        cfg = GLOBAL_CONFIG["attn"]
        qg, n = cs.shape[-2], cs.shape[-1]
        static, groups = self._static(cs.shape[1], qg, n)
        if top_p > 0.0:
            if cs.dtype != torch.bfloat16:
                raise ValueError(f"attn.top_p: the selection takes bfloat16 column sums (got {cs.dtype})")
            return ops.topk_mask_p(cs, topk, top_p, k_min, 0.01, groups, static, k_lens)
        if cs.is_cuda and amd_key("attn", "fused_topk_mask") and cs.dtype == torch.bfloat16 and n <= ops.TOPK_MASK_MAX_N:
            return ops.topk_mask(cs, topk, 0.01, groups, static, k_lens)
        mask = torch.randint(0, 100, cs.shape, device=cs.device, dtype=torch.uint8) == 0
        valid = _valid_keys(k_lens, n) if k_lens is not None else None
        if valid is not None:
            cs = cs.masked_fill(~valid, torch.finfo(cs.dtype).min)
        mask.scatter_(-1, cs.topk(k=topk, dim=-1).indices, True)
        mask.logical_and_(groups)
        mask.logical_or_(static)
        if valid is not None:
            mask.logical_and_(valid)
        return mask
# ... 72 lines not shown
            if amd_key("attn", "fused_packed_mask_to_indices") and packed.is_cuda and shape[-1] % 8 == 0:
                if amd_key("attn", "sorted_indices"):
                    return ops.mask_to_sorted_indices(packed, shape, multiple_of, bm)
                return ops.packed_mask_to_indices(packed, shape, multiple_of, bm)
            return ops.mask_to_indices(ops.bitunpack(packed, shape), multiple_of, bm)
        return self.storage.get_indices(), self.storage.get_counts()

    def _fast_attention(self, q: Tensor, k: Tensor, v: Tensor, inference_step: int, do_full_step: bool,
                        k_lens: Optional[Tensor] = None) -> Tensor:
        cfg = GLOBAL_CONFIG["attn"]
        bm = cfg["mbm"]
        assert bm == 192, "The kernel was written for BM=192. You may need to change the kernel."
        do_padding = cfg["pad_qkv_before_kernel"]
        multiple_of = 128 if do_padding else cfg["counts_multiple_of"]

        tm = bool(q.is_cuda and amd_key("attn", "token_major_output"))
        use_ragged = self._ragged_enabled(q)
        if self.layer_num < cfg["first_n_dense_layers"]:
            o, _ = ops.dense_attn(q, k, v, tm, k_lens)
            return o

        if do_full_step:
            if inference_step == 0:
                o, lse = ops.dense_attn(q, k, v, tm, k_lens) if do_padding else _dense_attn_raw(q, k, v, tm, k_lens)
                lse[..., k.shape[-2]:, :] = 0
                self.storage.set_lse_constants(lse)
                return o

            ragged = None
            if inference_step == 1 or cfg["recompute_mask"]:
                prev_lse = self.storage.get_lse_constants()
                tk = int(multiple_of * round((cfg["top_keys"] * k.shape[-2]) / multiple_of))
                top_p, k_min = self._top_p(k.shape[-2], multiple_of)
                mask = bs = None
                if (q.is_cuda and cfg["should_compress_indices"] and tk > 0 and amd_key("attn", "fused_colsum_topk")
                        and amd_key("attn", "fused_topk_mask") and k.shape[-2] <= ops.TOPK_MASK_MAX_N):
                    static, groups = self._static(q.shape[1], _cdiv(q.shape[-2], bm), k.shape[-2])
                    if top_p > 0.0:
                        o, mask, lse = ops.dense_colsum_topk_mask_p(q, k, v, prev_lse, tk, top_p, k_min, 0.01, groups, static, tm, k_lens)
                    else:
                        o, mask, lse = ops.dense_colsum_topk_mask(q, k, v, prev_lse, tk, 0.01, groups, static, tm, k_lens)
                elif do_padding:
                    o, bs, lse = ops.dense_colsum_attn(q, k, v, prev_lse, tm, k_lens)
                elif k_lens is not None:
                    o, bs, lse = torch.ops.chipmunk.dense_colsum_attn_varlen(q, k, v, prev_lse, k_lens, tm)
                else:
                    o, bs, lse = (torch.ops.chipmunk.dense_colsum_attn_layout(q, k, v, prev_lse, True) if tm else
                                  torch.ops.chipmunk.dense_colsum_attn(q, k, v, prev_lse))
                lse[..., k.shape[-2]:, :] = 0
                self.storage.set_lse_constants(lse)
                if cfg["should_compress_indices"]:
                    if mask is not None:
                        pass
                    elif tk > 0:
                        mask = self.random_and_topk(bs, tk, top_p, k_min, k_lens)
                    else:
                        mask = self._static(bs.shape[1], bs.shape[-2], bs.shape[-1])[0]
                        if k_lens is not None:
                            mask = mask & _valid_keys(k_lens, mask.shape[-1])
                    packed, mask_shape = ops.bitpack(mask)
                    self.mask_shape[self.layer_counter.cur_model_invocation_per_step] = mask_shape
                    self.storage.set_indices(packed)
                    if use_ragged:
                        ragged = self._ragged_indices(packed, mask_shape, multiple_of, bm, mask)
                        ragged = (ragged[0], ragged[1], _cap_counts(ragged[2], k_lens))
                        self._remember_indices(None, ragged[2], ragged[:2])
                    else:
                        if mask.is_cuda and amd_key("attn", "fused_packed_mask_to_indices") and amd_key("attn", "sorted_indices"):
                            inds, counts = ops.mask_to_sorted_indices(mask, mask.shape, multiple_of, bm)
                        else:
                            inds, counts = ops.mask_to_indices(mask, multiple_of, bm)
                        counts = _cap_counts(counts, k_lens)
                        self._remember_indices(inds, counts)
                else:
                    kseq = k.shape[-2]
                    bs = bs[..., :_cdiv(kseq, bm), :kseq]
                    if k_lens is not None:
                        bs = bs.masked_fill(~_valid_keys(k_lens, kseq), torch.finfo(bs.dtype).min)
                    inds = torch.topk(bs, k=tk, dim=-1).indices
                    counts = torch.full((q.shape[0], q.shape[1], _cdiv(q.shape[-2], bm)), tk, device=q.device,
                                        dtype=torch.int32)
                    pad = torch.empty((*counts.shape, q.shape[-2] - tk), device=q.device, dtype=torch.int32)
                    inds = torch.cat([inds, pad], dim=-1).to(torch.int32)
                    self.storage.set_indices(inds)
# ... 61 lines not shown
```

chipmunk_amd/ops/__init__.py:

```python
from .mlp import run_e2e as mlp, GLU_ACTS
from .mlp import run_e2e_glu as mlp_glu, run_e2e_glu, mm1_glu
from .mlp import run_e2e_glu_fp8 as mlp_glu_fp8, run_e2e_glu_fp8, mm1_glu_fp8
from .indexed_io import (copy_indices, topk_indices, mask_to_indices, scatter_add, packed_mask_to_indices,
                         mask_to_sorted_indices, mask_to_ragged_indices, topk_mask, topk_mask_p, topk_indices_p, topk_delta_indices_p, manual_seed,
                         topk_group_delta_indices, topk_group_delta_indices_p, TOPK_MASK_MAX_N)
from .attn import compact_indices, csp_attn, csp_attn_inplace, csp_attn_out, csp_attn_out_ragged, dense_attn, dense_colsum_attn, dense_colsum_topk_mask, dense_colsum_topk_mask_p
from .patch import patchify, unpatchify, patchify_rope
from .bitpack import bitpack, bitunpack
from . import voxel
from .w8_linear import w8_linear
from .qkv import qkv_split_norm, residual_ln_modulate, residual_ln_modulate_f32, split_heads_rownorm, wan_rope_table

__all__ = ["mlp", "copy_indices", "topk_indices", "mask_to_indices", "scatter_add", "csp_attn", "dense_attn",
           "dense_colsum_attn", "patchify", "unpatchify", "patchify_rope", "bitpack", "bitunpack",
           "packed_mask_to_indices", "mask_to_sorted_indices", "csp_attn_inplace", "csp_attn_out", "topk_mask", "TOPK_MASK_MAX_N", "voxel", "manual_seed", "qkv_split_norm", "dense_colsum_topk_mask", "compact_indices", "csp_attn_out_ragged", "residual_ln_modulate", "residual_ln_modulate_f32",
           "split_heads_rownorm", "wan_rope_table", "mask_to_ragged_indices", "mlp_glu", "run_e2e_glu", "mm1_glu",
           "mlp_glu_fp8", "run_e2e_glu_fp8", "mm1_glu_fp8", "topk_mask_p", "dense_colsum_topk_mask_p",
           "topk_indices_p", "topk_delta_indices_p", "topk_group_delta_indices", "topk_group_delta_indices_p", "w8_linear"]

from . import _fake
```

chipmunk_amd/ops/_fake.py:

```python
import torch


def _o_like(q, token_major):
    B, H, N, D = q.shape
    return q.new_empty((B, N, H, D)).permute(0, 2, 1, 3) if token_major else q.new_empty((B, H, N, D))


def _register():
    lib = torch.library

    @lib.register_fake("chipmunk::csp_128_attn")
    def _(q, k, v, indices, indices_counts):
        return torch.empty_like(q)

    @lib.register_fake("chipmunk::csp_attn_out")
    def _(q, k, v, o_in, indices, indices_counts, o_scale):
        return torch.empty_like(o_in)

    @lib.register_fake("chipmunk::residual_ln_modulate")
    def _(x, y, gate, shift, scale, eps):
        return [torch.empty_like(x), torch.empty_like(x)] if y is not None else [torch.empty_like(x)]

    @lib.register_fake("chipmunk::residual_ln_modulate_f32")
    def _(x, y, gate, shift, scale, weight, bias, eps):
# ... 103 lines not shown
        G = (Nq + 191) // 192
        return [_o_like(q, token_major_o), q.new_empty((B, H, G, k.shape[2]), dtype=torch.bool),
                q.new_empty((B, H, Nq, 1), dtype=torch.float32)]

    def _dense_out(q):
        return q.new_empty((q.shape[0], q.shape[1], q.shape[2], 1), dtype=torch.float32)

    @lib.register_fake("chipmunk::dense_attn_varlen")
    def _(q, k, v, k_lens, token_major_o=False):
        return [_o_like(q, token_major_o), _dense_out(q)]

    @lib.register_fake("chipmunk::dense_colsum_attn_varlen")
    def _(q, k, v, p, k_lens, token_major_o=False):
        groups = (q.shape[2] + 191) // 192
        return [_o_like(q, token_major_o), q.new_empty((q.shape[0], q.shape[1], groups, max(q.shape[2], k.shape[2]))), _dense_out(q)]

    @lib.register_fake("chipmunk::topk_mask_varlen")
    def _(cs, k_lens, k, random_amount, groups, static_mask):
        return cs.new_empty(cs.shape, dtype=torch.bool)

    @lib.register_fake("chipmunk::topk_mask_p_varlen")
    def _(cs, k_lens, k, top_p, k_min, random_amount, groups, static_mask):
        return cs.new_empty(cs.shape, dtype=torch.bool)

    @lib.register_fake("chipmunk::dense_colsum_topk_mask_varlen")
    def _(q, k, v, p, k_lens, k_top, random_amount, groups, static_mask, token_major_o=False):
        G = (q.shape[2] + 191) // 192
        return [_o_like(q, token_major_o), q.new_empty((q.shape[0], q.shape[1], G, k.shape[2]), dtype=torch.bool), _dense_out(q)]

    @lib.register_fake("chipmunk::dense_colsum_topk_mask_p_varlen")
    def _(q, k, v, p, k_lens, k_top, top_p, k_min, random_amount, groups, static_mask, token_major_o=False):
        G = (q.shape[2] + 191) // 192
        return [_o_like(q, token_major_o), q.new_empty((q.shape[0], q.shape[1], G, k.shape[2]), dtype=torch.bool), _dense_out(q)]

    @lib.register_fake("chipmunk::topk_indices_p")
    def _(activation, indices, counts, sparsity_amount, top_p, min_keys, multiple_of, random_amount):
        torch._check(activation.ndim == 3 and activation.shape[-1] >= 1024, lambda: "activation must be [batch, rows, cols] with cols >= 1024")
        torch._check(indices.shape == activation.shape and counts.numel() == activation.shape[0] * activation.shape[1],
                     lambda: "indices must have the shape of activation, counts must be [batch, rows]")
        return None

    @lib.register_fake("chipmunk::topk_delta_indices_p")
    def _(activation, cache, indices, counts, sparsity_amount, top_p, min_keys, multiple_of, random_amount):
        torch._check(activation.ndim == 3 and activation.shape[-1] >= 1024, lambda: "activation must be [batch, rows, cols] with cols >= 1024")
        torch._check(cache.shape == activation.shape and cache.dtype == activation.dtype, lambda: "cache must have the shape and dtype of activation")
        torch._check(indices.shape == activation.shape and counts.numel() == activation.shape[0] * activation.shape[1],
                     lambda: "indices must have the shape of activation, counts must be [batch, rows]")
        return None

    def _check_group_delta(activation, cache, indices, counts, rows_per_group):
        torch._check(activation.ndim == 3 and activation.shape[-1] >= 1024, lambda: "activation must be [batch, rows, cols] with cols >= 1024")
        torch._check(cache.shape == activation.shape and cache.dtype == activation.dtype, lambda: "cache must have the shape and dtype of activation")
        torch._check(1 <= rows_per_group <= 64, lambda: "rows_per_group must be in [1, 64]")
        groups = (activation.shape[1] + rows_per_group - 1) // rows_per_group
        torch._check(tuple(indices.shape) == (activation.shape[0], groups, activation.shape[2]) and tuple(counts.shape) == (activation.shape[0], groups),
                     lambda: "indices must be [batch, ceil(rows / rows_per_group), cols], counts [batch, ceil(rows / rows_per_group)]")

    @lib.register_fake("chipmunk::topk_group_delta_indices")
    def _(activation, cache, indices, counts, rows_per_group, sparsity_amount, multiple_of, random_amount):
        _check_group_delta(activation, cache, indices, counts, rows_per_group)
        return None

    @lib.register_fake("chipmunk::topk_group_delta_indices_p")
    def _(activation, cache, indices, counts, rows_per_group, sparsity_amount, top_p, min_keys, multiple_of, random_amount):
        _check_group_delta(activation, cache, indices, counts, rows_per_group)
        return None
# ... 108 lines not shown
```

chipmunk_amd/ops/attn.py:

```python
from __future__ import annotations

from typing import Optional, Tuple

import torch
import torch.nn.functional as F

PM = 192


def _pad_len(n: int) -> int:
    return ((n + PM - 1) // PM) * PM


def _last_dim_contiguous(t: torch.Tensor) -> torch.Tensor:
    return t if t.stride(-1) == 1 else t.contiguous()


def check_k_lens(k_lens: Optional[torch.Tensor], like: torch.Tensor, who: str) -> Optional[torch.Tensor]:
    if k_lens is None:
        return None
    if not like.is_cuda:
        raise ValueError(f"{who}: k_lens is supported on the GPU only (got {like.device} operands)")
    if not isinstance(k_lens, torch.Tensor) or k_lens.dtype != torch.int32:
        raise ValueError(f"{who}: k_lens must be an int32 tensor (got {getattr(k_lens, 'dtype', type(k_lens))})")
# ... 12 lines not shown
    if check_k_lens(k_lens, q, "dense_attn") is not None:
        o, l = torch.ops.chipmunk.dense_attn_varlen(q, k, v, k_lens, token_major_o)
    else:
        o, l = torch.ops.chipmunk.dense_attn_layout(q, k, v, True) if token_major_o else torch.ops.chipmunk.dense_attn(q, k, v)
    padded = _pad_len(n)
    if padded != n:
        l = F.pad(l, (0, 0, 0, padded - n))
    return o, l


def dense_colsum_attn(q: torch.Tensor, k: torch.Tensor, v: torch.Tensor, p: torch.Tensor, token_major_o: bool = False,
                      k_lens: Optional[torch.Tensor] = None) -> Tuple[torch.Tensor, torch.Tensor, torch.Tensor]:
    n = q.shape[-2]
    padded = _pad_len(n)
    assert p.shape[-2] in (n, padded), "p must be the l vector of the previous full step"
    p_rows = p[..., :n, :].contiguous()
    q, k, v = _last_dim_contiguous(q), _last_dim_contiguous(k), _last_dim_contiguous(v)
    if check_k_lens(k_lens, q, "dense_colsum_attn") is not None:
        o, cs, l = torch.ops.chipmunk.dense_colsum_attn_varlen(q, k, v, p_rows, k_lens, token_major_o)
    elif token_major_o:
        o, cs, l = torch.ops.chipmunk.dense_colsum_attn_layout(q, k, v, p_rows, True)
    else:
        o, cs, l = torch.ops.chipmunk.dense_colsum_attn(q, k, v, p_rows)
    if padded != n:
        l = F.pad(l, (0, 0, 0, padded - n))
    kseq = k.shape[-2]
    kgroups = (kseq + PM - 1) // PM
    if cs.shape[-2] != kgroups or cs.shape[-1] != kseq:
        cs = cs[..., :kgroups, :kseq]
    return o, cs, l


def dense_colsum_topk_mask(q: torch.Tensor, k: torch.Tensor, v: torch.Tensor, p: torch.Tensor, k_top: int, random_amount: float,
                           groups, static_mask, token_major_o: bool = False, k_lens: Optional[torch.Tensor] = None
                           ) -> Tuple[torch.Tensor, torch.Tensor, torch.Tensor]:
    n = q.shape[-2]
    padded = _pad_len(n)
    assert p.shape[-2] in (n, padded), "p must be the l vector of the previous full step"
    if check_k_lens(k_lens, q, "dense_colsum_topk_mask") is not None:
        o, mask, l = torch.ops.chipmunk.dense_colsum_topk_mask_varlen(_last_dim_contiguous(q), _last_dim_contiguous(k), _last_dim_contiguous(v),
                                                                      p[..., :n, :].contiguous(), k_lens, k_top, random_amount, groups,
                                                                      static_mask, token_major_o)
    else:
        o, mask, l = torch.ops.chipmunk.dense_colsum_topk_mask(_last_dim_contiguous(q), _last_dim_contiguous(k), _last_dim_contiguous(v),
                                                               p[..., :n, :].contiguous(), k_top, random_amount, groups, static_mask,
                                                               token_major_o)
    if padded != n:
        l = F.pad(l, (0, 0, 0, padded - n))
    return o, mask, l


def dense_colsum_topk_mask_p(q: torch.Tensor, k: torch.Tensor, v: torch.Tensor, p: torch.Tensor, k_top: int, top_p: float, k_min: int,
                             random_amount: float, groups, static_mask, token_major_o: bool = False,
                             k_lens: Optional[torch.Tensor] = None) -> Tuple[torch.Tensor, torch.Tensor, torch.Tensor]:
    check_k_lens(k_lens, q, "dense_colsum_topk_mask_p")
    if not q.is_cuda:
        from .indexed_io import topk_mask_p
        o, cs, l = dense_colsum_attn(q, k, v, p, token_major_o)
        return o, topk_mask_p(cs, k_top, top_p, k_min, random_amount, groups, static_mask), l
    n = q.shape[-2]
    padded = _pad_len(n)
    assert p.shape[-2] in (n, padded), "p must be the l vector of the previous full step"
    if k_lens is not None:
        o, mask, l = torch.ops.chipmunk.dense_colsum_topk_mask_p_varlen(_last_dim_contiguous(q), _last_dim_contiguous(k),
                                                                        _last_dim_contiguous(v), p[..., :n, :].contiguous(), k_lens, k_top,
                                                                        top_p, k_min, random_amount, groups, static_mask, token_major_o)
    else:
        o, mask, l = torch.ops.chipmunk.dense_colsum_topk_mask_p(_last_dim_contiguous(q), _last_dim_contiguous(k), _last_dim_contiguous(v),
                                                                 p[..., :n, :].contiguous(), k_top, top_p, k_min, random_amount, groups,
                                                                 static_mask, token_major_o)
    if padded != n:
        l = F.pad(l, (0, 0, 0, padded - n))
    return o, mask, l


def csp_attn(q: torch.Tensor, k: torch.Tensor, v: torch.Tensor, indices: torch.Tensor,
             indices_counts: torch.Tensor) -> torch.Tensor:
    return torch.ops.chipmunk.csp_128_attn(q.contiguous(), k.contiguous(), v.contiguous(), indices.contiguous(),
                                           indices_counts.contiguous())


def csp_attn_inplace(q: torch.Tensor, k: torch.Tensor, v: torch.Tensor, o: torch.Tensor, indices: torch.Tensor,
                     indices_counts: torch.Tensor, o_scale: int) -> None:
    torch.ops.chipmunk.csp_attn(q, k, v, o, indices, indices_counts, o_scale)


def csp_attn_out(q: torch.Tensor, k: torch.Tensor, v: torch.Tensor, o_in: torch.Tensor, indices: torch.Tensor,
                 indices_counts: torch.Tensor, o_scale: int) -> torch.Tensor:
    return torch.ops.chipmunk.csp_attn_out(q, k, v, o_in, indices, indices_counts, o_scale)


def compact_indices(indices: torch.Tensor, indices_counts: torch.Tensor) -> Tuple[torch.Tensor, torch.Tensor]:
    return tuple(torch.ops.chipmunk.compact_indices(indices.contiguous(), indices_counts.contiguous()))


def csp_attn_out_ragged(q: torch.Tensor, k: torch.Tensor, v: torch.Tensor, o_in: torch.Tensor, indices: torch.Tensor,
                        offsets: torch.Tensor, indices_counts: torch.Tensor, o_scale: int) -> torch.Tensor:
    return torch.ops.chipmunk.csp_attn_out_ragged(q, k, v, o_in, indices, offsets, indices_counts, o_scale)


__all__ = ["csp_attn", "csp_attn_inplace", "csp_attn_out", "csp_attn_out_ragged", "compact_indices", "dense_attn", "dense_colsum_attn",
           "dense_colsum_topk_mask", "dense_colsum_topk_mask_p"]
```

chipmunk_amd/ops/indexed_io.py:

```python
from __future__ import annotations

from typing import List, Optional, Sequence

import torch

TOPK_MASK_MAX_N = 1024 * 512


def copy_indices(bm_fc1: torch.Tensor, bm_mid_cache: torch.Tensor, indices: torch.Tensor, counts: torch.Tensor) -> None:
    torch.ops.chipmunk.copy_indices(bm_fc1, bm_mid_cache, indices, counts)


def topk_indices(activations: torch.Tensor, indices_out: torch.Tensor, counts_out: torch.Tensor,
                 sparsity_amount: float, multiple_of: int, rk: float) -> None:
    torch.ops.chipmunk.topk_indices(activations, indices_out, counts_out, sparsity_amount, multiple_of, rk)


def _check_top_p(who: str, sparsity_amount: float, top_p: float, min_keys: float) -> None:
    if not (0.0 < top_p <= 1.0) or not (0.0 <= sparsity_amount <= 1.0) or not (0.0 <= min_keys <= 1.0 - sparsity_amount + 1e-9):
        raise ValueError(f"{who}: top_p must be in (0, 1], sparsity_amount in [0, 1] and min_keys in [0, 1 - sparsity_amount] "
                         f"(got top_p {top_p}, sparsity_amount {sparsity_amount}, min_keys {min_keys})")


def _f32(x: float) -> float:
    return float(torch.tensor(float(x), dtype=torch.float32))


def _topk_indices_p_cpu(activations: torch.Tensor, indices_out: torch.Tensor, counts_out: torch.Tensor, sparsity_amount: float,
                        top_p: float, min_keys: float, multiple_of: int, rk: float) -> None:
    f = activations.shape[-1]
    if f < 1024:
        raise ValueError(f"topk_indices_p: rows of 1024 columns or more (the quantiles are taken over the first 1024); got {f}")
    rows = activations.reshape(-1, f).double()
    inds, counts = indices_out.view(-1, f), counts_out.view(-1)
    if _f32(sparsity_amount) == 1.0:
# ... 125 lines not shown
    rank = (0xFFFF - _bf16_keys(cs).view(-1, n)) * (1 << 30) + ((cols % 4096) // 4) * (1 << 20) + cols
    order = torch.argsort(rank, dim=-1)
    val = cs.reshape(-1, n).double()
    mass = torch.where(val > 0, val, torch.zeros_like(val)).gather(-1, order)
    prefix = mass.cumsum(-1)
    total = prefix[:, -1:]
    k_p = (prefix < top_p * total).sum(-1) + 1
    k_p = torch.where(total[:, 0] > 0, k_p, torch.zeros_like(k_p))
    s = k_p.clamp(min=int(k_min)).clamp(max=k)
    keep = torch.zeros(cs.numel() // n, n, dtype=torch.bool)
    keep.scatter_(-1, order, cols[None, :] < s[:, None])
    keep = keep.view(B, H, G, n)
    if random_amount > 0:
        keep |= torch.rand(keep.shape) < random_amount
    if groups is not None:
        keep &= groups
    if static_mask is not None:
        keep = keep | static_mask
    return keep


def topk_mask_p(cs: torch.Tensor, k: int, top_p: float, k_min: int = 0, random_amount: float = 0.0,
                groups: Optional[torch.Tensor] = None, static_mask: Optional[torch.Tensor] = None,
                k_lens: Optional[torch.Tensor] = None) -> torch.Tensor:
    from .attn import check_k_lens
    check_k_lens(k_lens, cs, "topk_mask_p")
    if not cs.is_cuda:
        return _topk_mask_p_cpu(cs, k, top_p, k_min, random_amount, groups, static_mask)
    if k_lens is not None:
        return torch.ops.chipmunk.topk_mask_p_varlen(cs, k_lens, k, top_p, k_min, random_amount, groups, static_mask)
    return torch.ops.chipmunk.topk_mask_p(cs, k, top_p, k_min, random_amount, groups, static_mask)


def manual_seed(seed: int) -> None:
    from .._native import manual_seed as _seed
    _seed(seed)
```

chipmunk_amd/util/config.py:

```python
from __future__ import annotations

import copy
from typing import Any, Dict

import yaml

BASE_CONFIG: Dict[str, Any] = {
    "num_model_invocations_per_inference_step": 1,
    "should_profile": False,
    "generation_index": 0,
    "steps": 50,
    "world_size": 1,
    "mlp": {
        "is_enabled": True,
        "is_fp8": False,
        "top_keys": "dd",
        "random_keys": 0.05,
        "full_step_every": 10,
        "block_mask_cache": 2,
        "first_n_dense_layers": 2,
        "counts_multiple_of": 256,
        "bm": 128,
        "mbm": 128,
    },
# ... 25 lines not shown
        "mlp.sparse_act_T": False,
        "mlp.blockmean_mid_cache": False,
        "attn.out_cache": True,
        "attn.indices": True,
        "attn.counts": False,
        "attn.lse_constants": False,
        "text_encoders": True,
    },
    "step_caching": {
        "is_enabled": True,
        "skip_step_schedule": {7, 11, 13, 14, 15, 17, 18, 19, 21, 22, 23, 25, 26, 27, 29, 31, 33, 34, 35, 37, 38, 39,
                               41, 42, 43},
    },
}

AMD_EXTRA_KEYS: Dict[str, Any] = {
    "offloading.keep_resident_if_fits": False,
    "offloading.hbm_budget_gb": 200.0,
    "offloading.native_host_pool": True,
    "attn.fused_packed_mask_to_indices": True,
    "attn.sorted_indices": True,
    "mlp.fused_topk_delta": True,
    "mlp.fused_block_mean": True,
    "mlp.fused_fp8_quantize": True,
    "attn.fused_residual": True,
    "attn.fused_topk_mask": True,
    "attn.fused_colsum_topk": True,
    "mlp.fused_scatter": True,
    "attn.token_major_output": False,
    "attn.keep_unpacked_indices": True,
    "attn.keep_unpacked_indices_offloaded": True,
    "attn.kept_indices_offloaded_budget_gb": 8.0,
    "attn.ragged_mask_to_indices": True,
    "mlp.fp8_fc2": False,
    "mlp.fp8_weight_only": False,
    "mlp.w8_stream_rows": 0,
    "attn.top_p": 0.0,
    "attn.top_p_min_keys": 0.0,
    "mlp.top_p": 0.0,
    "mlp.top_p_min_keys": 0.0,
    "mlp.fp8_scaling": "tensor",
    "mlp.cache_layout": "column",
    "mlp.fused_group_topk_delta": False,
}
BASE_CONFIG["offloading"]["keep_resident_if_fits"] = AMD_EXTRA_KEYS["offloading.keep_resident_if_fits"]
BASE_CONFIG["offloading"]["hbm_budget_gb"] = AMD_EXTRA_KEYS["offloading.hbm_budget_gb"]
BASE_CONFIG["offloading"]["native_host_pool"] = AMD_EXTRA_KEYS["offloading.native_host_pool"]
BASE_CONFIG["attn"]["fused_packed_mask_to_indices"] = AMD_EXTRA_KEYS["attn.fused_packed_mask_to_indices"]
BASE_CONFIG["attn"]["sorted_indices"] = AMD_EXTRA_KEYS["attn.sorted_indices"]
BASE_CONFIG["mlp"]["fused_topk_delta"] = AMD_EXTRA_KEYS["mlp.fused_topk_delta"]
BASE_CONFIG["attn"]["fused_residual"] = AMD_EXTRA_KEYS["attn.fused_residual"]
BASE_CONFIG["attn"]["fused_topk_mask"] = AMD_EXTRA_KEYS["attn.fused_topk_mask"]
BASE_CONFIG["attn"]["fused_colsum_topk"] = AMD_EXTRA_KEYS["attn.fused_colsum_topk"]
BASE_CONFIG["mlp"]["fused_scatter"] = AMD_EXTRA_KEYS["mlp.fused_scatter"]
BASE_CONFIG["attn"]["token_major_output"] = AMD_EXTRA_KEYS["attn.token_major_output"]
BASE_CONFIG["attn"]["keep_unpacked_indices"] = AMD_EXTRA_KEYS["attn.keep_unpacked_indices"]
BASE_CONFIG["attn"]["keep_unpacked_indices_offloaded"] = AMD_EXTRA_KEYS["attn.keep_unpacked_indices_offloaded"]
BASE_CONFIG["attn"]["kept_indices_offloaded_budget_gb"] = AMD_EXTRA_KEYS["attn.kept_indices_offloaded_budget_gb"]
BASE_CONFIG["attn"]["ragged_mask_to_indices"] = AMD_EXTRA_KEYS["attn.ragged_mask_to_indices"]
BASE_CONFIG["mlp"]["fp8_fc2"] = AMD_EXTRA_KEYS["mlp.fp8_fc2"]
BASE_CONFIG["mlp"]["fp8_weight_only"] = AMD_EXTRA_KEYS["mlp.fp8_weight_only"]
BASE_CONFIG["mlp"]["w8_stream_rows"] = AMD_EXTRA_KEYS["mlp.w8_stream_rows"]
BASE_CONFIG["attn"]["top_p"] = AMD_EXTRA_KEYS["attn.top_p"]
BASE_CONFIG["attn"]["top_p_min_keys"] = AMD_EXTRA_KEYS["attn.top_p_min_keys"]
BASE_CONFIG["mlp"]["top_p"] = AMD_EXTRA_KEYS["mlp.top_p"]
BASE_CONFIG["mlp"]["top_p_min_keys"] = AMD_EXTRA_KEYS["mlp.top_p_min_keys"]
BASE_CONFIG["mlp"]["fp8_scaling"] = AMD_EXTRA_KEYS["mlp.fp8_scaling"]
BASE_CONFIG["mlp"]["cache_layout"] = AMD_EXTRA_KEYS["mlp.cache_layout"]
BASE_CONFIG["mlp"]["fused_group_topk_delta"] = AMD_EXTRA_KEYS["mlp.fused_group_topk_delta"]

GLOBAL_CONFIG: Dict[str, Any] = copy.deepcopy(BASE_CONFIG)


def amd_key(section: str, key: str) -> Any:
    return GLOBAL_CONFIG.get(section, {}).get(key, AMD_EXTRA_KEYS[f"{section}.{key}"])


def update_global_config(config: Dict[str, Any]) -> None:
    GLOBAL_CONFIG.update(config)


def _deep_update(dst: Dict[str, Any], src: Dict[str, Any]) -> None:
    for key, value in src.items():
        if isinstance(value, dict) and isinstance(dst.get(key), dict):
            _deep_update(dst[key], value)
        else:
            dst[key] = value


def load_from_file(config_file: str) -> None:
    with open(config_file, "r") as f:
        loaded = yaml.safe_load(f)
# ... 10 lines not shown
```

include/chipmunk_hip.h:

```cpp
#ifndef CHIPMUNK_HIP_H
#define CHIPMUNK_HIP_H

#include <stdint.h>

#ifdef __cplusplus
extern "C" {
#endif

#define CHIPMUNK_OK 0
#define CHIPMUNK_ERR_INVALID 1
#define CHIPMUNK_ERR_LAUNCH 2
#define CHIPMUNK_ERR_UNSUPPORTED 3

#define CHIPMUNK_DTYPE_BF16 0
#define CHIPMUNK_DTYPE_FP16 1
#define CHIPMUNK_DTYPE_FP32 2

const char *chipmunk_last_error(void);
int chipmunk_abi_version(void);
int chipmunk_set_option(const char *name, int value);
int chipmunk_set_random_seed(uint64_t seed);

int chipmunk_csp_attn(const void *q, const void *k, const void *v, void *o, const int64_t q_strides[3],
                      const int64_t k_strides[3], const int64_t v_strides[3], const int64_t o_strides[3],
// ... 232 lines not shown
                                      const int64_t *o_strides, void *cs, float *l, const int32_t *k_lens, int B, int H,
                                      int Nq, int Nk, int cs_stride, void *stream);
int chipmunk_dense_colsum_topk_mask_varlen(const void *q, const void *k, const void *v, const int64_t q_strides[3],
                                           const int64_t k_strides[3], const int64_t v_strides[3], const float *p, void *o,
                                           const int64_t *o_strides, float *l, const int32_t *k_lens, int B, int H, int Nq,
                                           int Nk, const void *static_mask, int64_t static_stride, int static_rows,
                                           const void *group_flags, void *mask, int k_top, double random_amount, void *stream);
int chipmunk_dense_colsum_topk_mask_p_varlen(const void *q, const void *k, const void *v, const int64_t q_strides[3],
                                             const int64_t k_strides[3], const int64_t v_strides[3], const float *p, void *o,
                                             const int64_t *o_strides, float *l, const int32_t *k_lens, int B, int H, int Nq,
                                             int Nk, const void *static_mask, int64_t static_stride, int static_rows,
                                             const void *group_flags, void *mask, int k_top, double random_amount,
                                             double top_p, int k_min, void *stream);
int chipmunk_topk_mask_varlen(const void *cs, int64_t cs_stride, const void *static_mask, int64_t static_stride,
                              int static_rows, const void *group_flags, void *mask, const int32_t *k_lens, int seq_rows,
                              int rows, int n, int k, double random_amount, void *stream);
int chipmunk_topk_mask_p_varlen(const void *cs, int64_t cs_stride, const void *static_mask, int64_t static_stride,
                                int static_rows, const void *group_flags, void *mask, const int32_t *k_lens, int seq_rows,
                                int rows, int n, int k, double random_amount, double top_p, int k_min, void *stream);

int chipmunk_mask_to_indices(const void *mask, int32_t *indices, int32_t *counts, int64_t rows, int n, int pad_n,
                             int multiple_of, void *stream);

int chipmunk_packed_mask_to_indices(const void *packed, int32_t *indices, int32_t *counts, int64_t rows, int n,
                                    int pad_n, int multiple_of, void *stream);

int chipmunk_mask_to_sorted_indices(const void *mask, int packed, int32_t *indices, int32_t *counts, int64_t rows,
                                    int n, int pad_n, int multiple_of, void *stream);

int chipmunk_mask_row_counts(const void *mask, int packed, int32_t *counts, int64_t *lengths, int64_t rows, int n, int pad_n,
                             int multiple_of, void *stream);
int chipmunk_mask_to_ragged_indices(const void *mask, int packed, int sorted, const int64_t *offsets, int32_t *flat, int64_t rows,
                                    int n, int multiple_of, void *stream);

int chipmunk_copy_indices(const void *src, void *dst, const int32_t *inds, const int32_t *counts, int B, int M, int R,
                          int F, int elem_size, void *stream);

int chipmunk_transpose16(const void *src, void *dst, int B, int R, int C, void *stream);
int chipmunk_transpose16_pitched(const void *src, void *dst, int B, int R, int C, int ld, void *stream);

int chipmunk_block_mean(const void *x, void *out, int64_t rows, int C, int mbm, void *stream);
int chipmunk_block_mean_ragged(const void *x, void *out, int64_t rows, int C, int mbm, void *stream);

int chipmunk_quantize_fp8(const void *x, const float *scale, void *out, int64_t n, float max_value, void *stream);

#define CHIPMUNK_QUANTIZE_ROWWISE_MAX_K 16384
int chipmunk_quantize_fp8_rowwise(const void *x, void *out, float *scale_recip, int64_t rows, int K, float max_value, void *stream);

int chipmunk_bitpack(const void *mask, void *packed, int64_t n, void *stream);
int chipmunk_bitunpack(const void *packed, void *mask, int64_t n, void *stream);

int chipmunk_gather_rows(const void *src, void *dst, const int32_t *map, int64_t outer, int64_t n_src, int64_t n_out,
                         int64_t row_bytes, void *stream);

int chipmunk_host_alloc(size_t bytes, void **host_ptr);
int chipmunk_host_free(void *host_ptr);
int chipmunk_copy_d2h_async(void *host_dst, const void *dev_src, size_t bytes, void *stream);
int chipmunk_copy_h2d_async(void *dev_dst, const void *host_src, size_t bytes, void *stream);
size_t chipmunk_host_bytes(void);

int chipmunk_release_scratch(void);
int chipmunk_big_scratch_fallbacks(void);

int chipmunk_qkv_split_norm(const void *qkv, int64_t row_stride, const void *q_weight, const void *k_weight, void *q, void *k,
                            void *v, int64_t n, int heads, float eps, const float *freqs_cos, const float *freqs_sin,
                            int64_t rope_rows, void *stream);
// ... 11 lines not shown
```

Measured before the change: 0.5784.

## Emit packed bit masks with per-row kept counts directly from top-k selection

Adds a BITS mode to the top-k mask kernels that writes one bit per key (assembled across lanes with DPP) instead of one byte, and records the number of kept keys per row. A new small kernel turns these counts into padded counts and lengths, so the later mask-to-indices step can skip a separate row-count pass. Static masks are read as packed bits too. The new path is on by default through attn.packed_selection. It cuts mask memory traffic and a pass over the mask, in exchange for more kernel variants and a requirement that the key count be a multiple of 8.

```diff
diff --git a/chipmunk_amd/_native.py b/chipmunk_amd/_native.py
--- a/chipmunk_amd/_native.py
+++ b/chipmunk_amd/_native.py
@@ -25,6 +25,7 @@
     "chipmunk_bitpack", "chipmunk_bitunpack", "chipmunk_transpose16", "chipmunk_block_mean", "chipmunk_quantize_fp8", "chipmunk_gather_rows", "chipmunk_qkv_split_norm", "chipmunk_split_heads_rownorm", "chipmunk_dense_colsum_topk_mask", "chipmunk_dense_attn_strided", "chipmunk_csp_attn_out_ragged", "chipmunk_compact_indices", "chipmunk_residual_ln_modulate", "chipmunk_residual_ln_modulate_f32", "chipmunk_dense_colsum_attn_strided", "chipmunk_dense_colsum_topk_mask_strided", "chipmunk_release_scratch", "chipmunk_big_scratch_fallbacks",
     "chipmunk_dense_attn_varlen", "chipmunk_dense_colsum_attn_varlen", "chipmunk_dense_colsum_topk_mask_varlen",
     "chipmunk_dense_colsum_topk_mask_p_varlen", "chipmunk_topk_mask_varlen", "chipmunk_topk_mask_p_varlen",
+    "chipmunk_topk_bits", "chipmunk_dense_colsum_topk_bits", "chipmunk_row_lengths_from_counts",
     "chipmunk_host_alloc", "chipmunk_host_free", "chipmunk_copy_d2h_async", "chipmunk_copy_h2d_async", "chipmunk_host_bytes",
 ]
 
diff --git a/chipmunk_amd/csrc/attn.hip b/chipmunk_amd/csrc/attn.hip
--- a/chipmunk_amd/csrc/attn.hip
+++ b/chipmunk_amd/csrc/attn.hip
@@ -1273,14 +1273,15 @@
                                        const int64_t *o_strides, float *l, int B, int H, int Nq, int Nk, const void *static_mask,
                                        int64_t static_stride, int static_rows, const void *group_flags, void *mask,
                                        int topk, double random_amount, bool mass, double top_p, int k_min, void *stream,
-                                       const int32_t *klens = nullptr) {
+                                       const int32_t *klens = nullptr, int32_t *row_counts = nullptr) {
     if (int e = check_common(q, k, v, o, B, H, Nq, Nk)) return e;
     CM_CHECK(l && pin && mask, "dense_colsum_topk_mask: p / l / mask missing");
     if (int e = check_strides(q_strides, "q")) return e;
     if (int e = check_strides(k_strides, "k")) return e;
     if (int e = check_strides(v_strides, "v")) return e;
     hipStream_t st = (hipStream_t)stream;
-    if (!use_dense64(B, H, Nq, Nk) || chipmunk_get_option("attn_fused_colsum") == 2 || (Nk & 3) || Nk > CHIPMUNK_TOPK_MASK_MAX_N)
+    if (!use_dense64(B, H, Nq, Nk) || chipmunk_get_option("attn_fused_colsum") == 2 || (Nk & 3) || Nk > CHIPMUNK_TOPK_MASK_MAX_N ||
+        (row_counts && (Nk & 7)))
         return CHIPMUNK_ERR_UNSUPPORTED;
     AttnParams p = {};
     p.q = (const uint16_t *)q, p.k = (const uint16_t *)k, p.v = (const uint16_t *)v, p.o = (uint16_t *)o;
@@ -1295,6 +1296,9 @@
     if (!part) return CHIPMUNK_ERR_UNSUPPORTED;
     if (int e = chipmunk_dense64_colsum_launch(p, part, st)) return e;
     const int nrb = ((Nq + 255) / 256) * 2;
+    if (row_counts)
+        return chipmunk_topk_bits_parts(part, chipmunk_colsum_part_stride(Nk), nrb, p.G, Nq, static_mask, static_stride, static_rows, group_flags, mask,
+                                        row_counts, B * H * p.G, Nk, topk, mass ? top_p : 0.0, k_min, random_amount, st, klens, H * p.G);
     if (mass)
         return chipmunk_topk_mask_p_parts(part, chipmunk_colsum_part_stride(Nk), nrb, p.G, Nq, static_mask, static_stride, static_rows, group_flags, mask,
                                           B * H * p.G, Nk, topk, top_p, k_min, random_amount, st, klens, H * p.G);
@@ -1330,6 +1334,18 @@
     return chipmunk_dense_colsum_topk_mask_strided(q, k, v, q_strides, k_strides, v_strides, pin, o, nullptr, l, B, H, Nq, Nk,
                                                    static_mask, static_stride, static_rows, group_flags, mask, topk, random_amount,
                                                    stream);
+}
+
+extern "C" int chipmunk_dense_colsum_topk_bits(const void *q, const void *k, const void *v, const int64_t q_strides[3],
+                                               const int64_t k_strides[3], const int64_t v_strides[3], const float *pin, void *o,
+                                               const int64_t *o_strides, float *l, const int32_t *k_lens, int B, int H, int Nq, int Nk,
+                                               const void *static_bits, int64_t static_stride, int static_rows, const void *group_flags,
+                                               void *packed, int32_t *row_counts, int topk, double random_amount, double top_p, int k_min,
+                                               void *stream) {
+    CM_CHECK(row_counts, "dense_colsum_topk_bits: counts missing");
+    CM_CHECK(top_p >= 0.0 && top_p <= 1.0 && k_min >= 0, "dense_colsum_topk_bits: top_p must be in [0, 1] and k_min >= 0 (got %g, %d)", top_p, k_min);
+    return dense_colsum_topk_mask_impl(q, k, v, q_strides, k_strides, v_strides, pin, o, o_strides, l, B, H, Nq, Nk, static_bits, static_stride,
+                                       static_rows, group_flags, packed, topk, random_amount, top_p > 0.0, top_p, k_min, stream, k_lens, row_counts);
 }
 
 extern "C" int chipmunk_dense_colsum_topk_mask_varlen(const void *q, const void *k, const void *v, const int64_t q_strides[3],
diff --git a/chipmunk_amd/csrc/attn_params.h b/chipmunk_amd/csrc/attn_params.h
--- a/chipmunk_amd/csrc/attn_params.h
+++ b/chipmunk_amd/csrc/attn_params.h
@@ -42,6 +42,9 @@
 int chipmunk_topk_mask_p_parts(const uint16_t *part, int part_stride, int nrb, int groups_per_bh, int Nq, const void *static_mask, int64_t static_stride,
                                int static_rows, const void *group_flags, void *mask, int rows, int n, int k, double top_p, int k_min,
                                double random_amount, hipStream_t stream, const int32_t *klens = nullptr, int seq_rows = 0);
+int chipmunk_topk_bits_parts(const uint16_t *part, int part_stride, int nrb, int groups_per_bh, int Nq, const void *static_bits, int64_t static_stride,
+                             int static_rows, const void *group_flags, void *packed, int32_t *row_counts, int rows, int n, int k, double top_p,
+                             int k_min, double random_amount, hipStream_t stream, const int32_t *klens = nullptr, int seq_rows = 0);
 size_t chipmunk_colsum_part_bytes(int B, int H, int Nq, int Nk);
 int chipmunk_colsum_part_stride(int Nk);
 int chipmunk_colsum64_launch(const AttnParams &p, hipStream_t stream);
diff --git a/chipmunk_amd/csrc/indexed_io.hip b/chipmunk_amd/csrc/indexed_io.hip
--- a/chipmunk_amd/csrc/indexed_io.hip
+++ b/chipmunk_amd/csrc/indexed_io.hip
@@ -246,6 +246,15 @@
     }
 }
 
+__global__ __launch_bounds__(256) void row_lengths_from_counts_kernel(const int32_t *kept, int32_t *counts, int64_t *lengths, int64_t rows,
+                                                                      int pad_n, int multiple_of) {
+    const int64_t row = (int64_t)blockIdx.x * 256 + threadIdx.x;
+    if (row >= rows) return;
+    const int64_t padded = (((int64_t)kept[row] + multiple_of - 1) / multiple_of) * multiple_of;
+    counts[row] = (int32_t)padded;
+    lengths[row] = (min(padded, (int64_t)pad_n) + 31) / 32 * 32;
+}
+
 struct TopkParams {
     const void *act;
     void *cache;
@@ -671,6 +680,7 @@
     int k_min;
     const int32_t *klens;
     int seq_rows;
+    int32_t *row_counts;
 };
 
 __device__ __forceinline__ int topk_mask_row_len(const TopkMaskParams &p, int row) {
@@ -716,8 +726,27 @@
     return (u & 0x8000u) ? (~u & 0xffffu) : (u | 0x8000u);
 }
 
-template <int KPT, bool ALIGNED, bool PARTS = false, bool MASS = false>
+__device__ __forceinline__ uint32_t nibbles_to_dword(uint32_t nib, int lane) {
+    uint32_t w = nib << (4 * (lane & 7));
+    w |= (uint32_t)__builtin_amdgcn_update_dpp(0, (int)w, 0xB1, 0xf, 0xf, true);
+    w |= (uint32_t)__builtin_amdgcn_update_dpp(0, (int)w, 0x4E, 0xf, 0xf, true);
+    w |= (uint32_t)__builtin_amdgcn_update_dpp(0, (int)w, 0x141, 0xf, 0xf, true);
+    return w;
+}
+typedef uint32_t __attribute__((aligned(1))) u32_unaligned;
+__device__ __forceinline__ void store_row_bits(uint8_t *out, int byte, int nb, uint32_t w) {
+    if (byte + 4 <= nb) {
+        *(u32_unaligned *)(out + byte) = w;
+    } else {
+#pragma unroll
+        for (int i = 0; i < 3; ++i)
+            if (byte + i < nb) out[byte + i] = (uint8_t)(w >> (8 * i));
+    }
+}
+
+template <int KPT, bool ALIGNED, bool PARTS = false, bool MASS = false, bool BITS = false>
 __global__ __launch_bounds__(1024) void topk_mask_kernel(const TopkMaskParams p) {
+    static_assert(!BITS || ALIGNED, "the packed output stage is built for the aligned form");
     constexpr int NV = KPT / 4;
     __shared__ int wave_cnt[16];
     const int tid = threadIdx.x, lane = tid & 63, w = tid >> 6;
@@ -926,7 +955,7 @@
         __syncthreads();
         tie_budget = ties_to_take - before;
     }
-    uint8_t *out = p.mask + (int64_t)row * n;
+    uint8_t *out = p.mask + (BITS ? ((int64_t)row * n) >> 3 : (int64_t)row * n);
     const uint8_t *st = p.stat ? p.stat + (int64_t)(row % p.stat_rows) * p.stat_stride : nullptr;
     const bool rnd = active && p.random_amount > 0.f;
     auto combined4 = [&](int c0, uint32_t &v0, uint32_t &v1) {
@@ -951,7 +980,8 @@
     }
     const uint32_t salt = p.salt ^ (first * 0x27D4EB2Fu);
     const int nsteps = (n + 4095) / 4096;
-    auto emit = [&](auto keyed, int c, uint32_t v0, uint32_t v1, uint32_t sb) {
+    constexpr int W = BITS ? 1 : 8;
+    auto keep4 = [&](auto keyed, int c, uint32_t v0, uint32_t v1, uint32_t sb) {
         uint32_t bytes = 0;
         if constexpr (decltype(keyed)::value) asm volatile("" : "+v"(v0), "+v"(v1));
 #pragma unroll
@@ -963,10 +993,14 @@
             tie_budget -= tie ? 1 : 0;
             keep = keep || tie;
             if (rnd && !keep) keep = hash_uniform(row, c + e, salt) < p.random_amount;
-            keep = keep || ((sb >> (8 * e)) & 0xffu) != 0;
+            keep = keep || ((sb >> (W * e)) & (BITS ? 1u : 0xffu)) != 0;
             keep = keep && c + e < nv;
-            bytes |= (keep ? 1u : 0u) << (8 * e);
-        }
+            bytes |= (keep ? 1u : 0u) << (W * e);
+        }
+        return bytes;
+    };
+    auto emit = [&](auto keyed, int c, uint32_t v0, uint32_t v1, uint32_t sb) {
+        const uint32_t bytes = keep4(keyed, c, v0, v1, sb);
         if constexpr (ALIGNED) {
             *(uint32_t *)(out + c) = bytes;
         } else {
@@ -975,7 +1009,35 @@
                 if (c + e < n) out[c + e] = (uint8_t)(bytes >> (8 * e));
         }
     };
-    if constexpr (ALIGNED) {
+    if constexpr (BITS) {
+        constexpr int OB = 5;
+        int kept = 0;
+#pragma unroll
+        for (int j0 = 0; j0 < NV; j0 += OB) {
+            uint32_t sbv[OB];
+#pragma unroll
+            for (int jj = 0; jj < OB; ++jj) {
+                const int c = 4 * tid + 4096 * (j0 + jj);
+                sbv[jj] = (j0 + jj < NV && st && c < n) ? (uint32_t)st[c >> 3] : 0u;
+            }
+            __builtin_amdgcn_sched_barrier(0);
+#pragma unroll
+            for (int jj = 0; jj < OB; ++jj) {
+                const int j = j0 + jj < NV ? j0 + jj : 0, c = 4 * tid + 4096 * (j0 + jj);
+                if (j0 + jj < NV && 4096 * (j0 + jj) < n) {
+                    uint32_t nib = 0;
+                    if (c < n) nib = keep4(std::integral_constant<int, 1>{}, c, key[j][0], key[j][1], (sbv[jj] >> (c & 4)) & 15u);
+                    kept += __popc(nib);
+                    const uint32_t w8 = nibbles_to_dword(nib, lane);
+                    if ((lane & 7) == 0) store_row_bits(out, c >> 3, n >> 3, w8);
+                }
+                asm volatile("" ::: "memory");
+            }
+            __builtin_amdgcn_sched_barrier(0);
+        }
+        kept = block_count(kept);
+        if (tid == 0) p.row_counts[row] = kept;
+    } else if constexpr (ALIGNED) {
         constexpr int OB = 5;
 #pragma unroll
         for (int j0 = 0; j0 < NV; j0 += OB) {
@@ -1020,8 +1082,9 @@
     return u ^ (s | 0x80008000u);
 }
 
-template <bool ALIGNED, bool PARTS, bool MASS = false>
+template <bool ALIGNED, bool PARTS, bool MASS = false, bool BITS = false>
 __global__ __launch_bounds__(1024) void topk_mask_stream_kernel(const TopkMaskParams p) {
+    static_assert(!BITS || ALIGNED, "the packed output stage is built for the aligned form");
     __shared__ int wave_cnt[16];
     const int tid = threadIdx.x, lane = tid & 63, w = tid >> 6;
     const int row = blockIdx.x;
@@ -1240,7 +1303,9 @@
         __syncthreads();
         tie_budget = ties_to_take - before;
     }
-    uint8_t *out = p.mask + (int64_t)row * n;
+    uint8_t *out = p.mask + (BITS ? ((int64_t)row * n) >> 3 : (int64_t)row * n);
+    constexpr int W = BITS ? 1 : 8;
+    int kept = 0;
     const uint8_t *st = p.stat ? p.stat + (int64_t)(row % p.stat_rows) * p.stat_stride : nullptr;
     for (int j0 = 0; j0 < nsteps; j0 += U) {
         uint32_t kw[U][2], sbv[U];
@@ -1250,7 +1315,9 @@
             kw[jj][0] = kw[jj][1] = 0;
             if (select) load_raw(j0 + jj, kw[jj][0], kw[jj][1]);
             sbv[jj] = 0;
-            if constexpr (ALIGNED) {
+            if constexpr (BITS) {
+                if (st && c < n) sbv[jj] = ((uint32_t)st[c >> 3] >> (c & 4)) & 15u;
+            } else if constexpr (ALIGNED) {
                 if (st && c < n) sbv[jj] = *(const uint32_t *)(st + c);
             } else if (st) {
 #pragma unroll
@@ -1261,7 +1328,7 @@
 #pragma unroll
         for (int jj = 0; jj < U; ++jj) {
             const int c = 4 * tid + 4096 * (j0 + jj);
-            if (c >= n) continue;
+            if (BITS ? 4096 * (j0 + jj) >= n : c >= n) continue;
             if (select) to_keys(kw[jj][0], kw[jj][1]);
             uint32_t bytes = 0;
 #pragma unroll
@@ -1272,11 +1339,15 @@
                 tie_budget -= tie ? 1 : 0;
                 keep = keep || tie;
                 if (rnd && !keep) keep = hash_uniform(row, c + e, salt) < p.random_amount;
-                keep = keep || ((sbv[jj] >> (8 * e)) & 0xffu) != 0;
+                keep = keep || ((sbv[jj] >> (W * e)) & (BITS ? 1u : 0xffu)) != 0;
                 keep = keep && c + e < nv;
-                bytes |= (keep ? 1u : 0u) << (8 * e);
-            }
-            if constexpr (ALIGNED) {
+                bytes |= (keep ? 1u : 0u) << (W * e);
+            }
+            if constexpr (BITS) {
+                kept += __popc(bytes);
+                const uint32_t w8 = nibbles_to_dword(bytes, lane);
+                if ((lane & 7) == 0) store_row_bits(out, c >> 3, n >> 3, w8);
+            } else if constexpr (ALIGNED) {
                 *(uint32_t *)(out + c) = bytes;
             } else {
 #pragma unroll
@@ -1284,6 +1355,10 @@
                     if (c + e < n) out[c + e] = (uint8_t)(bytes >> (8 * e));
             }
         }
+    }
+    if constexpr (BITS) {
+        kept = block_count(kept);
+        if (tid == 0) p.row_counts[row] = kept;
     }
 }
 
@@ -1406,6 +1481,19 @@
     return CHIPMUNK_OK;
 }
 
+extern "C" int chipmunk_row_lengths_from_counts(const int32_t *kept, int32_t *counts, int64_t *lengths, int64_t rows, int n, int pad_n,
+                                                int multiple_of, void *stream) {
+    CM_CHECK(kept && counts && lengths, "row_lengths_from_counts: null pointer");
+    CM_CHECK(rows >= 0 && rows < (1ll << 31) && n > 0 && pad_n >= n && multiple_of > 0, "row_lengths_from_counts: bad sizes rows=%lld n=%d pad_n=%d multiple_of=%d",
+             (long long)rows, n, pad_n, multiple_of);
+    CM_CHECK(m2i_lds_bytes(n, true) <= 160 * 1024, "mask_to_indices: row length %d needs %zu B of LDS (> 160 KiB)", n, m2i_lds_bytes(n, true));
+    if (rows == 0) return CHIPMUNK_OK;
+    hipLaunchKernelGGL(row_lengths_from_counts_kernel, dim3((unsigned)((rows + 255) / 256)), dim3(256), 0, (hipStream_t)stream, kept, counts,
+                       lengths, rows, pad_n, multiple_of);
+    CM_LAUNCH_CHECK();
+    return CHIPMUNK_OK;
+}
+
 extern "C" int chipmunk_mask_to_ragged_indices(const void *mask, int packed, int sorted, const int64_t *offsets, int32_t *flat,
                                                int64_t rows, int n, int multiple_of, void *stream) {
     if (packed) return sorted ? launch_m2i<true, true, true>(mask, flat, nullptr, rows, n, n, multiple_of, stream, offsets)
@@ -1551,15 +1639,21 @@
     return CHIPMUNK_OK;
 }
 
-template <bool MASS>
+template <bool MASS, bool BITS = false>
 static int topk_mask_parts_impl(const uint16_t *part, int part_stride, int nrb, int groups_per_bh, int Nq, const void *static_mask, int64_t static_stride,
                                 int static_rows, const void *group_flags, void *mask, int rows, int n, int k, double random_amount,
-                                double top_p, int k_min, hipStream_t s, const int32_t *klens, int seq_rows) {
+                                double top_p, int k_min, hipStream_t s, const int32_t *klens, int seq_rows, int32_t *row_counts = nullptr) {
     CM_CHECK(!klens || seq_rows > 0, "topk_mask_parts: k_lens without the rows per sequence");
     CM_CHECK(part && mask && rows >= 0 && n > 0 && (n & 3) == 0 && n <= CHIPMUNK_TOPK_MASK_MAX_N && k >= 0 && part_stride >= n && (part_stride & 3) == 0, "topk_mask_parts: bad arguments");
-    CM_CHECK(!static_mask || (static_rows > 0 && static_stride >= n && (static_stride & 3) == 0 && ((uintptr_t)static_mask & 3) == 0),
-             "topk_mask_parts: bad static mask geometry");
-    CM_CHECK(((uintptr_t)mask & 3) == 0 && ((uintptr_t)part & 7) == 0, "topk_mask_parts: unaligned buffers");
+    if (BITS) {
+        CM_CHECK(row_counts && (n & 7) == 0, "topk_bits_parts: rows of a multiple of 8 columns and a counts buffer (n = %d)", n);
+        CM_CHECK(!static_mask || (static_rows > 0 && static_stride >= n / 8), "topk_bits_parts: bad static plane geometry");
+        CM_CHECK(((uintptr_t)part & 7) == 0, "topk_bits_parts: unaligned partial rows");
+    } else {
+        CM_CHECK(!static_mask || (static_rows > 0 && static_stride >= n && (static_stride & 3) == 0 && ((uintptr_t)static_mask & 3) == 0),
+                 "topk_mask_parts: bad static mask geometry");
+        CM_CHECK(((uintptr_t)mask & 3) == 0 && ((uintptr_t)part & 7) == 0, "topk_mask_parts: unaligned buffers");
+    }
     if (rows == 0) return CHIPMUNK_OK;
     TopkMaskParams p = {nullptr, (const uint8_t *)static_mask, (const uint8_t *)group_flags, (uint8_t *)mask, 0, static_stride,
                         rows, n, k, static_mask ? static_rows : 1, (float)random_amount,
@@ -1567,10 +1661,11 @@
     p.parts = part, p.pstride = part_stride, p.nrb = nrb, p.ngroups = groups_per_bh, p.nq = Nq;
     p.top_p = (float)top_p, p.k_min = k_min;
     p.klens = klens, p.seq_rows = seq_rows;
-    if (n > 1024 * 120 || chipmunk_get_option("topk_mask_stream") == 1) hipLaunchKernelGGL((topk_mask_stream_kernel<true, true, MASS>), dim3(rows), dim3(1024), 0, s, p);
-    else if (n <= 1024 * 16) hipLaunchKernelGGL((topk_mask_kernel<16, true, true, MASS>), dim3(rows), dim3(1024), 0, s, p);
-    else if (n <= 1024 * 48) hipLaunchKernelGGL((topk_mask_kernel<48, true, true, MASS>), dim3(rows), dim3(1024), 0, s, p);
-    else hipLaunchKernelGGL((topk_mask_kernel<120, true, true, MASS>), dim3(rows), dim3(1024), 0, s, p);
+    p.row_counts = row_counts;
+    if (n > 1024 * 120 || chipmunk_get_option("topk_mask_stream") == 1) hipLaunchKernelGGL((topk_mask_stream_kernel<true, true, MASS, BITS>), dim3(rows), dim3(1024), 0, s, p);
+    else if (n <= 1024 * 16) hipLaunchKernelGGL((topk_mask_kernel<16, true, true, MASS, BITS>), dim3(rows), dim3(1024), 0, s, p);
+    else if (n <= 1024 * 48) hipLaunchKernelGGL((topk_mask_kernel<48, true, true, MASS, BITS>), dim3(rows), dim3(1024), 0, s, p);
+    else hipLaunchKernelGGL((topk_mask_kernel<120, true, true, MASS, BITS>), dim3(rows), dim3(1024), 0, s, p);
     CM_LAUNCH_CHECK();
     return CHIPMUNK_OK;
 }
@@ -1588,6 +1683,17 @@
     CM_CHECK(top_p > 0.0 && top_p <= 1.0 && k_min >= 0, "topk_mask_p_parts: top_p must be in (0, 1] and k_min >= 0 (got %g, %d)", top_p, k_min);
     return topk_mask_parts_impl<true>(part, part_stride, nrb, groups_per_bh, Nq, static_mask, static_stride, static_rows, group_flags, mask, rows, n, k,
                                       random_amount, top_p, k_min, s, klens, seq_rows);
+}
+
+int chipmunk_topk_bits_parts(const uint16_t *part, int part_stride, int nrb, int groups_per_bh, int Nq, const void *static_bits, int64_t static_stride,
+                             int static_rows, const void *group_flags, void *packed, int32_t *row_counts, int rows, int n, int k, double top_p,
+                             int k_min, double random_amount, hipStream_t s, const int32_t *klens, int seq_rows) {
+    CM_CHECK(top_p >= 0.0 && top_p <= 1.0 && k_min >= 0, "topk_bits_parts: top_p must be in [0, 1] and k_min >= 0 (got %g, %d)", top_p, k_min);
+    if (top_p > 0.0)
+        return topk_mask_parts_impl<true, true>(part, part_stride, nrb, groups_per_bh, Nq, static_bits, static_stride, static_rows, group_flags, packed,
+                                                rows, n, k, random_amount, top_p, k_min, s, klens, seq_rows, row_counts);
+    return topk_mask_parts_impl<false, true>(part, part_stride, nrb, groups_per_bh, Nq, static_bits, static_stride, static_rows, group_flags, packed,
+                                             rows, n, k, random_amount, 0.0, 0, s, klens, seq_rows, row_counts);
 }
 
 __global__ __launch_bounds__(256) void qkv_split_norm_kernel(const uint16_t *qkv, int64_t row_stride, const uint16_t *qw,
@@ -1690,6 +1796,46 @@
     return CHIPMUNK_OK;
 }
 
+template <bool MASS>
+static int topk_bits_impl(const void *cs, int64_t cs_stride, const void *static_bits, int64_t static_stride, int static_rows,
+                          const void *group_flags, void *packed, int32_t *row_counts, const int32_t *klens, int seq_rows, int rows, int n,
+                          int k, double random_amount, double top_p, int k_min, void *stream) {
+    CM_CHECK(cs && packed && row_counts, "topk_bits: null pointer");
+    CM_CHECK(!klens || (seq_rows > 0 && rows % seq_rows == 0), "topk_bits: %d rows are no whole sequences of %d rows", rows, seq_rows);
+    CM_CHECK(rows >= 0 && n > 0 && k >= 0, "topk_bits: bad sizes (rows=%d n=%d k=%d)", rows, n, k);
+    CM_CHECK(n % 8 == 0, "topk_bits: rows must be whole bytes, n %% 8 == 0 (got %d)", n);
+    CM_CHECK(n <= CHIPMUNK_TOPK_MASK_MAX_N, "topk_bits: rows of more than %d columns are not supported (got %d)", CHIPMUNK_TOPK_MASK_MAX_N, n);
+    CM_CHECK(cs_stride >= n && (((uintptr_t)cs) & 7) == 0 && cs_stride % 4 == 0, "topk_bits: cs rows must start on 8-byte boundaries (stride %lld)",
+             (long long)cs_stride);
+    CM_CHECK(!static_bits || (static_rows > 0 && static_stride >= n / 8), "topk_bits: bad static plane geometry");
+    CM_CHECK(random_amount >= 0.0 && random_amount <= 1.0, "topk_bits: random_amount must be in [0,1]");
+    if (rows == 0) return CHIPMUNK_OK;
+    TopkMaskParams p = {(const uint16_t *)cs, (const uint8_t *)static_bits, (const uint8_t *)group_flags, (uint8_t *)packed,
+                        cs_stride, static_stride, rows, n, k, static_bits ? static_rows : 1, (float)random_amount,
+                        random_amount > 0.0 ? chipmunk_next_random_salt() : 0u};
+    p.top_p = (float)top_p, p.k_min = k_min;
+    p.klens = klens, p.seq_rows = seq_rows;
+    p.row_counts = row_counts;
+    hipStream_t s = (hipStream_t)stream;
+    if (n > 1024 * 120 || chipmunk_get_option("topk_mask_stream") == 1) hipLaunchKernelGGL((topk_mask_stream_kernel<true, false, MASS, true>), dim3(rows), dim3(1024), 0, s, p);
+    else if (n <= 1024 * 16) hipLaunchKernelGGL((topk_mask_kernel<16, true, false, MASS, true>), dim3(rows), dim3(1024), 0, s, p);
+    else if (n <= 1024 * 48) hipLaunchKernelGGL((topk_mask_kernel<48, true, false, MASS, true>), dim3(rows), dim3(1024), 0, s, p);
+    else hipLaunchKernelGGL((topk_mask_kernel<120, true, false, MASS, true>), dim3(rows), dim3(1024), 0, s, p);
+    CM_LAUNCH_CHECK();
+    return CHIPMUNK_OK;
+}
+
+extern "C" int chipmunk_topk_bits(const void *cs, int64_t cs_stride, const void *static_bits, int64_t static_stride, int static_rows,
+                                  const void *group_flags, void *packed, int32_t *row_counts, const int32_t *k_lens, int seq_rows, int rows,
+                                  int n, int k, double random_amount, double top_p, int k_min, void *stream) {
+    CM_CHECK(top_p >= 0.0 && top_p <= 1.0 && k_min >= 0, "topk_bits: top_p must be in [0, 1] and k_min >= 0 (got %g, %d)", top_p, k_min);
+    if (top_p > 0.0)
+        return topk_bits_impl<true>(cs, cs_stride, static_bits, static_stride, static_rows, group_flags, packed, row_counts, k_lens, seq_rows, rows, n,
+                                    k, random_amount, top_p, k_min, stream);
+    return topk_bits_impl<false>(cs, cs_stride, static_bits, static_stride, static_rows, group_flags, packed, row_counts, k_lens, seq_rows, rows, n, k,
+                                 random_amount, 0.0, 0, stream);
+}
+
 extern "C" int chipmunk_topk_mask(const void *cs, int64_t cs_stride, const void *static_mask, int64_t static_stride,
                                   int static_rows, const void *group_flags, void *mask, int rows, int n, int k,
                                   double random_amount, void *stream) {
diff --git a/chipmunk_amd/csrc/torch_registry.cpp b/chipmunk_amd/csrc/torch_registry.cpp
--- a/chipmunk_amd/csrc/torch_registry.cpp
+++ b/chipmunk_amd/csrc/torch_registry.cpp
@@ -1137,6 +1137,19 @@
     return {indices, counts};
 }
 
+static std::vector<at::Tensor> ragged_rows(const at::Tensor &mask, bool packed, bool sorted, const at::Tensor &counts, const at::Tensor &len,
+                                           int64_t rows, int64_t n, int64_t multiple_of) {
+    at::Tensor offsets = at::zeros({rows + 1}, len.options());
+    if (rows) offsets.narrow(0, 1, rows).copy_(len.cumsum(0));
+    const int64_t total = rows ? offsets[rows].item<int64_t>() : 0;
+    at::Tensor flat = at::empty({total + 64}, counts.options());
+    flat.narrow(0, total, 64).zero_();
+    check(chipmunk_mask_to_ragged_indices(mask.data_ptr(), packed ? 1 : 0, sorted ? 1 : 0, offsets.data_ptr<int64_t>(), flat.data_ptr<int>(),
+                                          rows, (int)n, (int)multiple_of, cur_stream(mask)),
+          "mask_to_ragged_indices");
+    return {flat, offsets, counts};
+}
+
 std::vector<at::Tensor> mask_to_ragged_indices(at::Tensor mask, at::IntArrayRef shape, int64_t multiple_of, int64_t pad_to_multiple_of,
                                                bool sorted) {
     CHECK_DEV(mask);
@@ -1156,15 +1169,29 @@
     check(chipmunk_mask_row_counts(mask.data_ptr(), packed ? 1 : 0, counts.data_ptr<int>(), len.data_ptr<int64_t>(), rows, (int)n,
                                    (int)pad_n, (int)multiple_of, cur_stream(mask)),
           "mask_to_ragged_indices");
-    at::Tensor offsets = at::zeros({rows + 1}, len.options());
-    if (rows) offsets.narrow(0, 1, rows).copy_(len.cumsum(0));
-    const int64_t total = rows ? offsets[rows].item<int64_t>() : 0;
-    at::Tensor flat = at::empty({total + 64}, counts.options());
-    flat.narrow(0, total, 64).zero_();
-    check(chipmunk_mask_to_ragged_indices(mask.data_ptr(), packed ? 1 : 0, sorted ? 1 : 0, offsets.data_ptr<int64_t>(), flat.data_ptr<int>(),
-                                          rows, (int)n, (int)multiple_of, cur_stream(mask)),
-          "mask_to_ragged_indices");
-    return {flat, offsets, counts};
+    return ragged_rows(mask, packed, sorted, counts, len, rows, n, multiple_of);
+}
+
+std::vector<at::Tensor> mask_to_ragged_indices_counted(at::Tensor packed, at::IntArrayRef shape, at::Tensor kept, int64_t multiple_of,
+                                                       int64_t pad_to_multiple_of, bool sorted) {
+    CHECK_DEV(packed); CHECK_DEV(kept);
+    TORCH_CHECK(packed.scalar_type() == at::kByte, "packed must be a uint8 bit-packed mask");
+    TORCH_CHECK(multiple_of > 0 && pad_to_multiple_of > 0, "multiple_of and pad_to_multiple_of must be positive");
+    TORCH_CHECK(shape.size() == 4, "shape must be [b, h, m, n]");
+    const int64_t b = shape[0], h = shape[1], m = shape[2], n = shape[3], rows = b * h * m;
+    TORCH_CHECK(n > 0 && n % 8 == 0 && packed.numel() * 8 >= rows * n, "bad packed mask");
+    TORCH_CHECK(kept.scalar_type() == at::kInt && kept.numel() == rows, "counts must be int32 with one entry per mask row");
+    const int64_t pad_n = ((n + pad_to_multiple_of - 1) / pad_to_multiple_of) * pad_to_multiple_of;
+    TORCH_CHECK(pad_n <= INT_MAX, "rows must have between 1 and 2^31 - 1 columns");
+    packed = packed.contiguous();
+    kept = kept.contiguous();
+    c10::DeviceGuard guard(packed.device());
+    at::Tensor counts = at::empty({b, h, m}, kept.options());
+    at::Tensor len = at::empty({rows}, kept.options().dtype(at::kLong));
+    check(chipmunk_row_lengths_from_counts(kept.data_ptr<int>(), counts.data_ptr<int>(), len.data_ptr<int64_t>(), rows, (int)n, (int)pad_n,
+                                           (int)multiple_of, cur_stream(packed)),
+          "mask_to_ragged_indices_counted");
+    return ragged_rows(packed, true, sorted, counts, len, rows, n, multiple_of);
 }
 
 std::vector<at::Tensor> dense_colsum_attn_layout(at::Tensor q, at::Tensor k, at::Tensor v, at::Tensor p, bool token_major_o);
@@ -1314,6 +1341,120 @@
     return topk_mask_impl(cs, k, true, top_p, k_min, random_amount, groups, static_mask);
 }
 
+struct BitsOperands {
+    const void *st = nullptr, *gf = nullptr;
+    int64_t st_stride = 0, st_rows = 1;
+    at::Tensor gfc;
+    bool ok = true;
+};
+static BitsOperands bits_operands(const c10::optional<at::Tensor> &groups, const c10::optional<at::Tensor> &static_bits, int64_t B, int64_t H,
+                                  int64_t G, int64_t N) {
+    BitsOperands r;
+    if (static_bits.has_value() && static_bits->defined()) {
+        const at::Tensor &sb = *static_bits;
+        r.ok = sb.is_cuda() && sb.scalar_type() == at::kByte && sb.dim() == 2 && sb.size(0) == G && sb.size(1) * 8 == N && sb.stride(1) == 1;
+        if (r.ok) r.st = sb.data_ptr(), r.st_stride = sb.stride(0), r.st_rows = G;
+    }
+    if (r.ok && groups.has_value() && groups->defined()) {
+        r.gfc = *groups;
+        r.ok = r.gfc.is_cuda() && r.gfc.scalar_type() == at::kBool && r.gfc.dim() == 4 && r.gfc.size(3) == 1 && r.gfc.size(2) == G &&
+               r.gfc.size(1) == H && (r.gfc.size(0) == 1 || r.gfc.size(0) == B);
+        if (r.ok) {
+            r.gfc = r.gfc.expand({B, H, G, 1}).contiguous();
+            r.gf = r.gfc.data_ptr();
+        }
+    }
+    return r;
+}
+
+static std::vector<at::Tensor> topk_bits_impl(at::Tensor cs, int64_t k, double top_p, int64_t k_min, double random_amount,
+                                              const c10::optional<at::Tensor> &groups, const c10::optional<at::Tensor> &static_bits,
+                                              const OptTensor &k_lens) {
+    CHECK_DEV(cs); CHECK_BF16(cs);
+    TORCH_CHECK(cs.dim() == 4 && cs.stride(3) == 1, "cs must be [B, H, G, N] with a contiguous last dim");
+    const int64_t B = cs.size(0), H = cs.size(1), G = cs.size(2), N = cs.size(3);
+    TORCH_CHECK(N % 8 == 0, "topk_bits: rows must be whole bytes, N % 8 == 0 (got ", N, ")");
+    TORCH_CHECK(top_p >= 0.0 && top_p <= 1.0 && k_min >= 0, "top_p must be in [0, 1] and k_min >= 0 (got ", top_p, ", ", k_min, ")");
+    const int32_t *kl = klens_ptr(k_lens, cs, B);
+    if (!(cs.stride(1) == G * cs.stride(2) && (B == 1 || cs.stride(0) == H * cs.stride(1)) && cs.stride(2) % 4 == 0 &&
+          ((uintptr_t)cs.data_ptr() & 7) == 0))
+        cs = cs.contiguous();
+    const int64_t rows = B * H * G;
+    c10::DeviceGuard guard(cs.device());
+    const BitsOperands ops = bits_operands(groups, static_bits, B, H, G, N);
+    TORCH_CHECK(ops.ok, "static_bits must be a uint8 bit-packed plane [G, N/8], groups bool [1|B, H, G, 1], both on the GPU");
+    at::Tensor packed = at::empty({rows * N / 8}, cs.options().dtype(at::kByte));
+    at::Tensor counts = at::empty({B, H, G}, cs.options().dtype(at::kInt));
+    check(chipmunk_topk_bits(cs.data_ptr(), cs.stride(2), ops.st, ops.st_stride, (int)ops.st_rows, ops.gf, packed.data_ptr(), counts.data_ptr<int>(),
+                             kl, (int)(H * G), (int)rows, (int)N, (int)k, random_amount, top_p, (int)(k_min > N ? N : k_min), cur_stream(cs)),
+          "topk_bits");
+    return {packed, counts};
+}
+
+std::vector<at::Tensor> topk_bits(at::Tensor cs, int64_t k, double random_amount, const c10::optional<at::Tensor> &groups,
+                                  const c10::optional<at::Tensor> &static_bits, const c10::optional<at::Tensor> &k_lens) {
+    return topk_bits_impl(cs, k, 0.0, 0, random_amount, groups, static_bits, k_lens);
+}
+
+std::vector<at::Tensor> topk_bits_p(at::Tensor cs, int64_t k, double top_p, int64_t k_min, double random_amount,
+                                    const c10::optional<at::Tensor> &groups, const c10::optional<at::Tensor> &static_bits,
+                                    const c10::optional<at::Tensor> &k_lens) {
+    TORCH_CHECK(top_p > 0.0, "topk_bits_p: top_p must be in (0, 1] (got ", top_p, ")");
+    return topk_bits_impl(cs, k, top_p, k_min, random_amount, groups, static_bits, k_lens);
+}
+
+static std::vector<at::Tensor> dense_colsum_topk_bits_impl(at::Tensor q, at::Tensor k, at::Tensor v, at::Tensor p, int64_t k_top, double top_p,
+                                                           int64_t k_min, double random_amount, const c10::optional<at::Tensor> &groups,
+                                                           const c10::optional<at::Tensor> &static_bits, bool token_major_o,
+                                                           const OptTensor &k_lens) {
+    const int32_t *kl = klens_ptr(k_lens, q, q.dim() == 4 ? q.size(0) : 0);
+    TORCH_CHECK(top_p >= 0.0 && top_p <= 1.0 && k_min >= 0, "top_p must be in [0, 1] and k_min >= 0 (got ", top_p, ", ", k_min, ")");
+    CHECK_DEV(q); CHECK_DEV(k); CHECK_DEV(v); CHECK_DEV(p);
+    CHECK_BF16(q); CHECK_BF16(k); CHECK_BF16(v);
+    TORCH_CHECK(q.dim() == 4 && k.dim() == 4 && k.size(2) % 8 == 0, "dense_colsum_topk_bits: q, k [B, H, N, 128] with a key count that is a multiple of 8");
+    const int64_t B = q.size(0), H = q.size(1), Nq = q.size(2), Nk = k.size(2), G = (Nq + 191) / 192;
+    const bool shapes_ok = v.dim() == 4 && q.size(3) == 128 && q.stride(3) == 1 && k.stride(3) == 1 && v.stride(3) == 1 &&
+                           p.scalar_type() == at::kFloat && p.is_contiguous() && p.numel() == B * H * Nq;
+    if (shapes_ok) {
+        const BitsOperands ops = bits_operands(groups, static_bits, B, H, G, Nk);
+        if (ops.ok) {
+            c10::DeviceGuard guard(q.device());
+            at::Tensor o = alloc_o(q, q, token_major_o);
+            const int64_t os[3] = {o.stride(0), o.stride(1), o.stride(2)};
+            at::Tensor l = at::empty({B, H, Nq, 1}, q.options().dtype(at::kFloat));
+            at::Tensor packed = at::empty({B * H * G * Nk / 8}, q.options().dtype(at::kByte));
+            at::Tensor counts = at::empty({B, H, G}, q.options().dtype(at::kInt));
+            const int64_t qs[3] = {q.stride(0), q.stride(1), q.stride(2)}, ks[3] = {k.stride(0), k.stride(1), k.stride(2)},
+                          vs[3] = {v.stride(0), v.stride(1), v.stride(2)};
+            const int rc = chipmunk_dense_colsum_topk_bits(q.data_ptr(), k.data_ptr(), v.data_ptr(), qs, ks, vs, p.data_ptr<float>(), o.data_ptr(), os,
+                                                           l.data_ptr<float>(), kl, (int)B, (int)H, (int)Nq, (int)Nk, ops.st, ops.st_stride,
+                                                           (int)ops.st_rows, ops.gf, packed.data_ptr(), counts.data_ptr<int>(), (int)k_top, random_amount,
+                                                           top_p, (int)(k_min > Nk ? Nk : k_min), cur_stream(q));
+            if (rc == CHIPMUNK_OK) return {o, packed, counts, l};
+            if (rc != CHIPMUNK_ERR_UNSUPPORTED) check(rc, "dense_colsum_topk_bits");
+        }
+    }
+    auto ocl = dense_colsum_attn_klens(q, k, v, p, token_major_o, k_lens);
+    at::Tensor cs = ocl[1];
+    if (cs.size(-1) != Nk || cs.size(-2) != G) cs = cs.slice(-2, 0, G).slice(-1, 0, Nk);
+    auto pc = topk_bits_impl(cs, k_top, top_p, k_min, random_amount, groups, static_bits, k_lens);
+    return {ocl[0], pc[0], pc[1], ocl[2]};
+}
+
+std::vector<at::Tensor> dense_colsum_topk_bits(at::Tensor q, at::Tensor k, at::Tensor v, at::Tensor p, int64_t k_top, double random_amount,
+                                               const c10::optional<at::Tensor> &groups, const c10::optional<at::Tensor> &static_bits,
+                                               bool token_major_o, const c10::optional<at::Tensor> &k_lens) {
+    return dense_colsum_topk_bits_impl(q, k, v, p, k_top, 0.0, 0, random_amount, groups, static_bits, token_major_o, k_lens);
+}
+
+std::vector<at::Tensor> dense_colsum_topk_bits_p(at::Tensor q, at::Tensor k, at::Tensor v, at::Tensor p, int64_t k_top, double top_p, int64_t k_min,
+                                                 double random_amount, const c10::optional<at::Tensor> &groups,
+                                                 const c10::optional<at::Tensor> &static_bits, bool token_major_o,
+                                                 const c10::optional<at::Tensor> &k_lens) {
+    TORCH_CHECK(top_p > 0.0, "dense_colsum_topk_bits_p: top_p must be in (0, 1] (got ", top_p, ")");
+    return dense_colsum_topk_bits_impl(q, k, v, p, k_top, top_p, k_min, random_amount, groups, static_bits, token_major_o, k_lens);
+}
+
 at::Tensor bitpack(at::Tensor mask) {
     TORCH_CHECK(mask.scalar_type() == at::kBool, "mask must be bool type");
     CHECK_DEV(mask);
@@ -1482,6 +1623,11 @@
     m.def("dense_colsum_topk_mask_p_varlen(Tensor q, Tensor k, Tensor v, Tensor p, Tensor k_lens, int k_top, float top_p, int k_min, float random_amount, Tensor? groups, Tensor? static_mask, bool token_major_o=False) -> Tensor[]");
     m.def("compact_indices(Tensor indices, Tensor counts) -> Tensor[]");
     m.def("mask_to_ragged_indices(Tensor mask, int[] shape, int multiple_of, int pad_to_multiple_of, bool sorted) -> Tensor[]");
+    m.def("mask_to_ragged_indices_counted(Tensor packed, int[] shape, Tensor counts, int multiple_of, int pad_to_multiple_of, bool sorted) -> Tensor[]");
+    m.def("topk_bits(Tensor cs, int k, float random_amount, Tensor? groups, Tensor? static_bits, Tensor? k_lens) -> Tensor[]");
+    m.def("topk_bits_p(Tensor cs, int k, float top_p, int k_min, float random_amount, Tensor? groups, Tensor? static_bits, Tensor? k_lens) -> Tensor[]");
+    m.def("dense_colsum_topk_bits(Tensor q, Tensor k, Tensor v, Tensor p, int k_top, float random_amount, Tensor? groups, Tensor? static_bits, bool token_major_o, Tensor? k_lens) -> Tensor[]");
+    m.def("dense_colsum_topk_bits_p(Tensor q, Tensor k, Tensor v, Tensor p, int k_top, float top_p, int k_min, float random_amount, Tensor? groups, Tensor? static_bits, bool token_major_o, Tensor? k_lens) -> Tensor[]");
     m.def("csp_attn_out_ragged(Tensor q, Tensor k, Tensor v, Tensor o_in, Tensor indices, Tensor offsets, Tensor indices_counts, int o_scale) -> Tensor");
     m.def("residual_ln_modulate(Tensor x, Tensor? y, Tensor? gate, Tensor shift, Tensor scale, float eps) -> Tensor[]");
     m.def("residual_ln_modulate_f32(Tensor x, Tensor? y, Tensor? gate, Tensor? shift, Tensor? scale, Tensor? weight, Tensor? bias, float eps) -> Tensor[]");
@@ -1547,6 +1693,11 @@
     m.impl("packed_mask_to_indices", &packed_mask_to_indices);
     m.impl("mask_to_sorted_indices", &mask_to_sorted_indices);
     m.impl("mask_to_ragged_indices", &mask_to_ragged_indices);
+    m.impl("mask_to_ragged_indices_counted", &mask_to_ragged_indices_counted);
+    m.impl("topk_bits", &topk_bits);
+    m.impl("topk_bits_p", &topk_bits_p);
+    m.impl("dense_colsum_topk_bits", &dense_colsum_topk_bits);
+    m.impl("dense_colsum_topk_bits_p", &dense_colsum_topk_bits_p);
     m.impl("topk_mask", &topk_mask);
     m.impl("topk_mask_p", &topk_mask_p);
     m.impl("transpose_last2", &transpose_last2);
diff --git a/chipmunk_amd/modules/attn.py b/chipmunk_amd/modules/attn.py
--- a/chipmunk_amd/modules/attn.py
+++ b/chipmunk_amd/modules/attn.py
@@ -15,6 +15,18 @@
 
 singleton_static_mask: Optional[Tensor] = None
 singleton_video_query_groups: Optional[Tensor] = None
+_static_plane_bits: Optional[Tuple[Optional[Tensor], Optional[Tensor]]] = None
+
+
+def packed_static_plane() -> Optional[Tensor]:
+    global _static_plane_bits
+    m = singleton_static_mask
+    if _static_plane_bits is None or _static_plane_bits[0] is not m:
+        plane = None
+        if m is not None and m.dim() == 4 and m.shape[0] == 1 and m.shape[-1] % 8 == 0 and bool((m == m[:, :1]).all()):
+            plane = ops.pack_static_plane(m[0, 0])
+        _static_plane_bits = (m, plane)
+    return _static_plane_bits[1]
 
 
 def _cdiv(a: int, b: int) -> int:
@@ -60,11 +72,13 @@
             for qg in range(n_video // 192):
                 centre = qg * 192 + 96
                 mask[qg, max(0, centre - window // 2):min(n_video, centre + window // 2)] = True
+        plane = ops.pack_static_plane(mask) if mask.shape[-1] % 8 == 0 else None
         mask = mask[None, None, :, :].expand(1, local_heads_num, -1, -1).contiguous()
         sparse_groups = (mask.sum(dim=-1, keepdim=True) + topk) < (n_video + txt_len)
-        global singleton_static_mask, singleton_video_query_groups
+        global singleton_static_mask, singleton_video_query_groups, _static_plane_bits
         singleton_static_mask = mask
         singleton_video_query_groups = sparse_groups
+        _static_plane_bits = (mask, plane)
 
     def _static(self, heads: int, qg: int, n: int):
         g0 = self.query_group_offset
@@ -73,6 +87,13 @@
             "(local_heads_num): build the static mask for the largest head chunk")
         h = min(heads, singleton_static_mask.shape[1])
         return (singleton_static_mask[:, :h, g0:g0 + qg, :n], singleton_video_query_groups[:, :h, g0:g0 + qg, :])
+
+    def _static_bits(self, qg: int, n: int) -> Optional[Tensor]:
+        plane = packed_static_plane()
+        g0 = self.query_group_offset
+        if plane is None or n % 8 != 0 or n // 8 > plane.shape[1] or g0 + qg > plane.shape[0]:
+            return None
+        return plane[g0:g0 + qg, :n // 8]
 
     @staticmethod
     def _top_p(n_keys: int, multiple_of: int):
@@ -211,11 +232,21 @@
                 prev_lse = self.storage.get_lse_constants()
                 tk = int(multiple_of * round((cfg["top_keys"] * k.shape[-2]) / multiple_of))
                 top_p, k_min = self._top_p(k.shape[-2], multiple_of)
-                mask = bs = None
+                mask = bs = packed = None
                 if (q.is_cuda and cfg["should_compress_indices"] and tk > 0 and amd_key("attn", "fused_colsum_topk")
                         and amd_key("attn", "fused_topk_mask") and k.shape[-2] <= ops.TOPK_MASK_MAX_N):
                     static, groups = self._static(q.shape[1], _cdiv(q.shape[-2], bm), k.shape[-2])
-                    if top_p > 0.0:
+                    sbits = None
+                    if use_ragged and amd_key("attn", "packed_selection"):
+                        sbits = self._static_bits(_cdiv(q.shape[-2], bm), k.shape[-2])
+                    if sbits is not None:
+                        mask_shape = torch.Size((q.shape[0], q.shape[1], _cdiv(q.shape[-2], bm), k.shape[-2]))
+                        if top_p > 0.0:
+                            o, (packed, kept), lse = ops.dense_colsum_topk_mask_p(q, k, v, prev_lse, tk, top_p, k_min, 0.01, groups, static, tm, k_lens,
+                                                                                  static_bits=sbits)
+                        else:
+                            o, (packed, kept), lse = ops.dense_colsum_topk_mask(q, k, v, prev_lse, tk, 0.01, groups, static, tm, k_lens, static_bits=sbits)
+                    elif top_p > 0.0:
                         o, mask, lse = ops.dense_colsum_topk_mask_p(q, k, v, prev_lse, tk, top_p, k_min, 0.01, groups, static, tm, k_lens)
                     else:
                         o, mask, lse = ops.dense_colsum_topk_mask(q, k, v, prev_lse, tk, 0.01, groups, static, tm, k_lens)
@@ -228,7 +259,13 @@
                                   torch.ops.chipmunk.dense_colsum_attn(q, k, v, prev_lse))
                 lse[..., k.shape[-2]:, :] = 0
                 self.storage.set_lse_constants(lse)
-                if cfg["should_compress_indices"]:
+                if packed is not None:
+                    self.mask_shape[self.layer_counter.cur_model_invocation_per_step] = mask_shape
+                    self.storage.set_indices(packed)
+                    ragged = ops.mask_to_ragged_indices_counted(packed, mask_shape, kept, multiple_of, bm, bool(amd_key("attn", "sorted_indices")))
+                    ragged = (ragged[0], ragged[1], _cap_counts(ragged[2], k_lens))
+                    self._remember_indices(None, ragged[2], ragged[:2])
+                elif cfg["should_compress_indices"]:
                     if mask is not None:
                         pass
                     elif tk > 0:
diff --git a/chipmunk_amd/ops/__init__.py b/chipmunk_amd/ops/__init__.py
--- a/chipmunk_amd/ops/__init__.py
+++ b/chipmunk_amd/ops/__init__.py
@@ -3,8 +3,9 @@
 from .mlp import run_e2e_glu_fp8 as mlp_glu_fp8, run_e2e_glu_fp8, mm1_glu_fp8
 from .indexed_io import (copy_indices, topk_indices, mask_to_indices, scatter_add, packed_mask_to_indices,
                          mask_to_sorted_indices, mask_to_ragged_indices, topk_mask, topk_mask_p, topk_indices_p, topk_delta_indices_p, manual_seed,
-                         topk_group_delta_indices, topk_group_delta_indices_p, TOPK_MASK_MAX_N)
-from .attn import compact_indices, csp_attn, csp_attn_inplace, csp_attn_out, csp_attn_out_ragged, dense_attn, dense_colsum_attn, dense_colsum_topk_mask, dense_colsum_topk_mask_p
+                         topk_group_delta_indices, topk_group_delta_indices_p, TOPK_MASK_MAX_N,
+                         topk_bits, topk_bits_p, pack_static_plane, mask_to_ragged_indices_counted)
+from .attn import compact_indices, csp_attn, csp_attn_inplace, csp_attn_out, csp_attn_out_ragged, dense_attn, dense_colsum_attn, dense_colsum_topk_mask, dense_colsum_topk_mask_p, dense_colsum_topk_bits, dense_colsum_topk_bits_p
 from .patch import patchify, unpatchify, patchify_rope
 from .bitpack import bitpack, bitunpack
 from . import voxel
@@ -16,6 +17,7 @@
            "packed_mask_to_indices", "mask_to_sorted_indices", "csp_attn_inplace", "csp_attn_out", "topk_mask", "TOPK_MASK_MAX_N", "voxel", "manual_seed", "qkv_split_norm", "dense_colsum_topk_mask", "compact_indices", "csp_attn_out_ragged", "residual_ln_modulate", "residual_ln_modulate_f32",
            "split_heads_rownorm", "wan_rope_table", "mask_to_ragged_indices", "mlp_glu", "run_e2e_glu", "mm1_glu",
            "mlp_glu_fp8", "run_e2e_glu_fp8", "mm1_glu_fp8", "topk_mask_p", "dense_colsum_topk_mask_p",
-           "topk_indices_p", "topk_delta_indices_p", "topk_group_delta_indices", "topk_group_delta_indices_p", "w8_linear"]
+           "topk_indices_p", "topk_delta_indices_p", "topk_group_delta_indices", "topk_group_delta_indices_p", "w8_linear",
+           "topk_bits", "topk_bits_p", "pack_static_plane", "mask_to_ragged_indices_counted", "dense_colsum_topk_bits", "dense_colsum_topk_bits_p"]
 
 from . import _fake
diff --git a/chipmunk_amd/ops/_fake.py b/chipmunk_amd/ops/_fake.py
--- a/chipmunk_amd/ops/_fake.py
+++ b/chipmunk_amd/ops/_fake.py
@@ -159,6 +159,28 @@
     def _(q, k, v, p, k_lens, k_top, top_p, k_min, random_amount, groups, static_mask, token_major_o=False):
         G = (q.shape[2] + 191) // 192
         return [_o_like(q, token_major_o), q.new_empty((q.shape[0], q.shape[1], G, k.shape[2]), dtype=torch.bool), _dense_out(q)]
+
+    def _bits_out(like, B, H, G, n):
+        torch._check(n % 8 == 0, lambda: "the key count must be a multiple of 8")
+        return [like.new_empty((B * H * G * n // 8,), dtype=torch.uint8), like.new_empty((B, H, G), dtype=torch.int32)]
+
+    @lib.register_fake("chipmunk::topk_bits")
+    def _(cs, k, random_amount, groups, static_bits, k_lens):
+        return _bits_out(cs, *cs.shape)
+
+    @lib.register_fake("chipmunk::topk_bits_p")
+    def _(cs, k, top_p, k_min, random_amount, groups, static_bits, k_lens):
+        return _bits_out(cs, *cs.shape)
+
+    @lib.register_fake("chipmunk::dense_colsum_topk_bits")
+    def _(q, k, v, p, k_top, random_amount, groups, static_bits, token_major_o, k_lens):
+        packed, counts = _bits_out(q, q.shape[0], q.shape[1], (q.shape[2] + 191) // 192, k.shape[2])
+        return [_o_like(q, token_major_o), packed, counts, _dense_out(q)]
+
+    @lib.register_fake("chipmunk::dense_colsum_topk_bits_p")
+    def _(q, k, v, p, k_top, top_p, k_min, random_amount, groups, static_bits, token_major_o, k_lens):
+        packed, counts = _bits_out(q, q.shape[0], q.shape[1], (q.shape[2] + 191) // 192, k.shape[2])
+        return [_o_like(q, token_major_o), packed, counts, _dense_out(q)]
 
     @lib.register_fake("chipmunk::topk_indices_p")
     def _(activation, indices, counts, sparsity_amount, top_p, min_keys, multiple_of, random_amount):
diff --git a/chipmunk_amd/ops/attn.py b/chipmunk_amd/ops/attn.py
--- a/chipmunk_amd/ops/attn.py
+++ b/chipmunk_amd/ops/attn.py
@@ -68,8 +68,11 @@
 
 
 def dense_colsum_topk_mask(q: torch.Tensor, k: torch.Tensor, v: torch.Tensor, p: torch.Tensor, k_top: int, random_amount: float,
-                           groups, static_mask, token_major_o: bool = False, k_lens: Optional[torch.Tensor] = None
-                           ) -> Tuple[torch.Tensor, torch.Tensor, torch.Tensor]:
+                           groups, static_mask, token_major_o: bool = False, k_lens: Optional[torch.Tensor] = None,
+                           static_bits: Optional[torch.Tensor] = None) -> Tuple[torch.Tensor, torch.Tensor, torch.Tensor]:
+    if static_bits is not None:
+        o, packed, counts, l = dense_colsum_topk_bits(q, k, v, p, k_top, random_amount, groups, static_bits, token_major_o, k_lens)
+        return o, (packed, counts), l
     n = q.shape[-2]
     padded = _pad_len(n)
     assert p.shape[-2] in (n, padded), "p must be the l vector of the previous full step"
@@ -88,7 +91,11 @@
 
 def dense_colsum_topk_mask_p(q: torch.Tensor, k: torch.Tensor, v: torch.Tensor, p: torch.Tensor, k_top: int, top_p: float, k_min: int,
                              random_amount: float, groups, static_mask, token_major_o: bool = False,
-                             k_lens: Optional[torch.Tensor] = None) -> Tuple[torch.Tensor, torch.Tensor, torch.Tensor]:
+                             k_lens: Optional[torch.Tensor] = None, static_bits: Optional[torch.Tensor] = None
+                             ) -> Tuple[torch.Tensor, torch.Tensor, torch.Tensor]:
+    if static_bits is not None:
+        o, packed, counts, l = dense_colsum_topk_bits_p(q, k, v, p, k_top, top_p, k_min, random_amount, groups, static_bits, token_major_o, k_lens)
+        return o, (packed, counts), l
     check_k_lens(k_lens, q, "dense_colsum_topk_mask_p")
     if not q.is_cuda:
         from .indexed_io import topk_mask_p
@@ -108,6 +115,35 @@
     if padded != n:
         l = F.pad(l, (0, 0, 0, padded - n))
     return o, mask, l
+
+
+def dense_colsum_topk_bits(q: torch.Tensor, k: torch.Tensor, v: torch.Tensor, p: torch.Tensor, k_top: int, random_amount: float,
+                           groups, static_bits, token_major_o: bool = False, k_lens: Optional[torch.Tensor] = None
+                           ) -> Tuple[torch.Tensor, torch.Tensor, torch.Tensor, torch.Tensor]:
+    return _dense_colsum_topk_bits(q, k, v, p, k_top, 0.0, 0, random_amount, groups, static_bits, token_major_o, k_lens)
+
+
+def dense_colsum_topk_bits_p(q: torch.Tensor, k: torch.Tensor, v: torch.Tensor, p: torch.Tensor, k_top: int, top_p: float, k_min: int,
+                             random_amount: float, groups, static_bits, token_major_o: bool = False,
+                             k_lens: Optional[torch.Tensor] = None) -> Tuple[torch.Tensor, torch.Tensor, torch.Tensor, torch.Tensor]:
+    return _dense_colsum_topk_bits(q, k, v, p, k_top, top_p, k_min, random_amount, groups, static_bits, token_major_o, k_lens)
+
+
+def _dense_colsum_topk_bits(q, k, v, p, k_top, top_p, k_min, random_amount, groups, static_bits, token_major_o, k_lens):
+    n = q.shape[-2]
+    padded = _pad_len(n)
+    assert p.shape[-2] in (n, padded), "p must be the l vector of the previous full step"
+    check_k_lens(k_lens, q, "dense_colsum_topk_bits")
+    q, k, v, p_rows = _last_dim_contiguous(q), _last_dim_contiguous(k), _last_dim_contiguous(v), p[..., :n, :].contiguous()
+    if top_p > 0.0:
+        o, packed, counts, l = torch.ops.chipmunk.dense_colsum_topk_bits_p(q, k, v, p_rows, k_top, top_p, k_min, random_amount, groups,
+                                                                           static_bits, token_major_o, k_lens)
+    else:
+        o, packed, counts, l = torch.ops.chipmunk.dense_colsum_topk_bits(q, k, v, p_rows, k_top, random_amount, groups, static_bits,
+                                                                         token_major_o, k_lens)
+    if padded != n:
+        l = F.pad(l, (0, 0, 0, padded - n))
+    return o, packed, counts, l
 
 
 def csp_attn(q: torch.Tensor, k: torch.Tensor, v: torch.Tensor, indices: torch.Tensor,
@@ -136,4 +172,4 @@
 
 
 __all__ = ["csp_attn", "csp_attn_inplace", "csp_attn_out", "csp_attn_out_ragged", "compact_indices", "dense_attn", "dense_colsum_attn",
-           "dense_colsum_topk_mask", "dense_colsum_topk_mask_p"]
+           "dense_colsum_topk_mask", "dense_colsum_topk_mask_p", "dense_colsum_topk_bits", "dense_colsum_topk_bits_p"]
diff --git a/chipmunk_amd/ops/indexed_io.py b/chipmunk_amd/ops/indexed_io.py
--- a/chipmunk_amd/ops/indexed_io.py
+++ b/chipmunk_amd/ops/indexed_io.py
@@ -1,6 +1,6 @@
 from __future__ import annotations
 
-from typing import List, Optional, Sequence
+from typing import List, Optional, Sequence, Tuple
 
 import torch
 
@@ -192,6 +192,36 @@
     return torch.ops.chipmunk.topk_mask_p(cs, k, top_p, k_min, random_amount, groups, static_mask)
 
 
+def topk_bits(cs: torch.Tensor, k: int, random_amount: float = 0.0, groups: Optional[torch.Tensor] = None,
+              static_bits: Optional[torch.Tensor] = None, k_lens: Optional[torch.Tensor] = None) -> Tuple[torch.Tensor, torch.Tensor]:
+    from .attn import check_k_lens
+    check_k_lens(k_lens, cs, "topk_bits")
+    packed, counts = torch.ops.chipmunk.topk_bits(cs, k, random_amount, groups, static_bits, k_lens)
+    return packed, counts
+
+
+def topk_bits_p(cs: torch.Tensor, k: int, top_p: float, k_min: int = 0, random_amount: float = 0.0,
+                groups: Optional[torch.Tensor] = None, static_bits: Optional[torch.Tensor] = None,
+                k_lens: Optional[torch.Tensor] = None) -> Tuple[torch.Tensor, torch.Tensor]:
+    from .attn import check_k_lens
+    check_k_lens(k_lens, cs, "topk_bits_p")
+    packed, counts = torch.ops.chipmunk.topk_bits_p(cs, k, top_p, k_min, random_amount, groups, static_bits, k_lens)
+    return packed, counts
+
+
+def pack_static_plane(plane: torch.Tensor) -> torch.Tensor:
+    from .bitpack import bitpack
+    g, n = plane.shape
+    if n % 8 != 0:
+        raise ValueError(f"pack_static_plane: the key count must be a multiple of 8 (got {n})")
+    return bitpack(plane.contiguous())[0].view(g, n // 8)
+
+
+def mask_to_ragged_indices_counted(packed: torch.Tensor, shape: Sequence[int], counts: torch.Tensor, multiple_of: int,
+                                   pad_to_multiple_of: int, sorted: bool = True) -> List[torch.Tensor]:
+    return torch.ops.chipmunk.mask_to_ragged_indices_counted(packed, list(shape), counts, multiple_of, pad_to_multiple_of, sorted)
+
+
 def manual_seed(seed: int) -> None:
     from .._native import manual_seed as _seed
     _seed(seed)
diff --git a/chipmunk_amd/util/config.py b/chipmunk_amd/util/config.py
--- a/chipmunk_amd/util/config.py
+++ b/chipmunk_amd/util/config.py
@@ -81,6 +81,7 @@
     "attn.keep_unpacked_indices_offloaded": True,
     "attn.kept_indices_offloaded_budget_gb": 8.0,
     "attn.ragged_mask_to_indices": True,
+    "attn.packed_selection": True,
     "mlp.fp8_fc2": False,
     "mlp.fp8_weight_only": False,
     "mlp.w8_stream_rows": 0,
@@ -107,6 +108,7 @@
 BASE_CONFIG["attn"]["keep_unpacked_indices_offloaded"] = AMD_EXTRA_KEYS["attn.keep_unpacked_indices_offloaded"]
 BASE_CONFIG["attn"]["kept_indices_offloaded_budget_gb"] = AMD_EXTRA_KEYS["attn.kept_indices_offloaded_budget_gb"]
 BASE_CONFIG["attn"]["ragged_mask_to_indices"] = AMD_EXTRA_KEYS["attn.ragged_mask_to_indices"]
+BASE_CONFIG["attn"]["packed_selection"] = AMD_EXTRA_KEYS["attn.packed_selection"]
 BASE_CONFIG["mlp"]["fp8_fc2"] = AMD_EXTRA_KEYS["mlp.fp8_fc2"]
 BASE_CONFIG["mlp"]["fp8_weight_only"] = AMD_EXTRA_KEYS["mlp.fp8_weight_only"]
 BASE_CONFIG["mlp"]["w8_stream_rows"] = AMD_EXTRA_KEYS["mlp.w8_stream_rows"]
diff --git a/include/chipmunk_hip.h b/include/chipmunk_hip.h
--- a/include/chipmunk_hip.h
+++ b/include/chipmunk_hip.h
@@ -288,6 +288,18 @@
                              int multiple_of, void *stream);
 int chipmunk_mask_to_ragged_indices(const void *mask, int packed, int sorted, const int64_t *offsets, int32_t *flat, int64_t rows,
                                     int n, int multiple_of, void *stream);
+int chipmunk_row_lengths_from_counts(const int32_t *kept, int32_t *counts, int64_t *lengths, int64_t rows, int n, int pad_n,
+                                     int multiple_of, void *stream);
+
+int chipmunk_topk_bits(const void *cs, int64_t cs_stride, const void *static_bits, int64_t static_stride, int static_rows,
+                       const void *group_flags, void *packed, int32_t *row_counts, const int32_t *k_lens, int seq_rows, int rows,
+                       int n, int k, double random_amount, double top_p, int k_min, void *stream);
+int chipmunk_dense_colsum_topk_bits(const void *q, const void *k, const void *v, const int64_t q_strides[3],
+                                    const int64_t k_strides[3], const int64_t v_strides[3], const float *p, void *o,
+                                    const int64_t *o_strides, float *l, const int32_t *k_lens, int B, int H, int Nq, int Nk,
+                                    const void *static_bits, int64_t static_stride, int static_rows, const void *group_flags,
+                                    void *packed, int32_t *row_counts, int k_top, double random_amount, double top_p, int k_min,
+                                    void *stream);
 
 int chipmunk_copy_indices(const void *src, void *dst, const int32_t *inds, const int32_t *counts, int B, int M, int R,
                           int F, int elem_size, void *stream);
```

New measurement: 0.5787, median of 2. No clear change (+0.1%).
